# DakeQQ/Automatic-Speech-Recognition-ASR-ONNX

Hardware: AMD Instinct MI355X
Metric: audio-sec/s, SenseVoiceSmall, 8 s @ 16 kHz chunks, batch 64 per GPU (RTF = 1/value per GPU-stream) (higher is better)
Workload: dtype bf16; 1 GPU; SenseVoiceSmall bf16 (234 M params, 70 SANM blocks), batch=64 x 8 s per GPU, greedy CTC; step k's audio is resident in HBM when the step starts, batch k+1's host->device copy (pinned, copy stream) and every token-id download are inside the timed region; global_batch=64, parallelism=dp1 (utterance sharding, RCCL arena broadcast + hypothesis gather)

## Files before the change

automatic-speech-recognition-asr-onnx_amd/_lib.py:

```python
from __future__ import annotations

import ctypes as C
import os
import subprocess

_HERE = os.path.dirname(os.path.abspath(__file__))
LIB_PATH = os.path.join(_HERE, "libasr_mi355x.so")
CSRC_DIR = os.path.join(_HERE, "csrc")

_lib = None


class AsrError(RuntimeError):
    def __init__(self, code: int, message: str):
        super().__init__(f"[asr_mi355x status {code}] {message}")
        self.code = code


class SenseVoiceConfigC(C.Structure):
    _fields_ = [(n, C.c_int32) for n in (
        "sample_rate", "n_mels", "nfft", "win_length", "hop_length", "lfr_m", "lfr_n", "d_model", "n_heads", "d_head",
        "d_ffn", "n_blocks", "n_main", "fsmn_kernel", "vocab", "blank_id", "n_prompt", "n_languages", "max_audio_len")] + [
        ("reserved", C.c_int32 * 8)]

# ... 20 lines not shown


_vp, _i, _sz = C.c_void_p, C.c_int, C.c_size_t
_fp, _ip, _lp, _dp = C.POINTER(C.c_float), C.POINTER(C.c_int32), C.POINTER(C.c_int64), C.POINTER(C.c_double)
SIGNATURES = {
    "asr_abi_version": (_i, []),
    "asr_last_error": (C.c_char_p, []),
    "asr_device_count": (_i, [C.POINTER(C.c_int)]),
    "asr_device_foreign_begin": (_i, [_i]),
    "asr_device_foreign_end": (_i, [_i]),
    "asr_device_foreign_stats": (_i, [_i, _lp]),
    "asr_sensevoice_create": (_i, [C.POINTER(SenseVoiceConfigC), _vp, _sz, _i, _i, _i, C.POINTER(_vp)]),
    "asr_sensevoice_run": (_i, [_vp, _vp, _i, _lp, _i, _ip, _ip, _i, _ip]),
    "asr_sensevoice_run_timed": (_i, [_vp, _vp, _i, _lp, _i, _ip, _ip, _i, _ip, _ip, _ip, _fp]),
    "asr_sensevoice_run_beam": (_i, [_vp, _vp, _i, _lp, _i, _ip, _i, _i, _i, _ip, _i, _ip, _fp, _fp]),
    "asr_sensevoice_set_hotwords": (_i, [_vp, _ip, _ip, _i, C.c_float]),
    "asr_sensevoice_set_lm": (_i, [_vp, _ip, C.c_int64, C.c_float, C.c_float, C.c_float]),
    "asr_sensevoice_align": (_i, [_vp, _vp, _i, _lp, _i, _ip, _ip, _ip, _ip, _ip, _fp, _fp, _fp, _ip]),
    "asr_sanm_stats": (_i, [_vp, _ip]),
    "asr_sensevoice_seq_len": (_i, [C.POINTER(SenseVoiceConfigC), _i, C.POINTER(C.c_int)]),
    "asr_paraformer_create": (_i, [C.POINTER(ParaformerConfigC), _vp, _sz, _i, _i, _i, C.POINTER(_vp)]),
    "asr_paraformer_run": (_i, [_vp, _vp, _i, _lp, _i, _ip, _i, _ip]),
    "asr_paraformer_run_timed": (_i, [_vp, _vp, _i, _lp, _i, _ip, _i, _ip, _ip, _fp]),
    "asr_paraformer_run_beam": (_i, [_vp, _vp, _i, _lp, _i, _i, _i, _i, _ip, _i, _ip, _fp, _fp, _ip, _fp]),
    "asr_paraformer_set_hotwords": (_i, [_vp, _ip, _ip, _i, C.c_float]),
    "asr_paraformer_set_lm": (_i, [_vp, _ip, C.c_int64, C.c_float, C.c_float, C.c_float]),
    "asr_paraformer_stream_create": (_i, [C.POINTER(ParaformerConfigC), _vp, _sz, _i, _i, _i, _i, _i, _i, _i, C.POINTER(_vp)]),
    "asr_paraformer_stream_reset": (_i, [_vp, _i]),
    "asr_paraformer_stream_step": (_i, [_vp, _vp, _i, _ip, _i, _ip, _i, _ip]),
    "asr_paraformer_stream_step_timed": (_i, [_vp, _vp, _i, _ip, _i, _ip, _i, _ip, _ip, _fp]),
    "asr_paraformer_stream_set_beam": (_i, [_vp, _i, _i, _i, _i]),
    "asr_paraformer_stream_set_hotwords": (_i, [_vp, _ip, _ip, _i, C.c_float]),
    "asr_paraformer_stream_set_lm": (_i, [_vp, _ip, C.c_int64, C.c_float, C.c_float, C.c_float]),
    "asr_paraformer_stream_step_beam": (_i, [_vp, _vp, _i, _ip, _i, _ip, _i, _ip, _ip, _fp, _ip, _fp, _ip, _ip, _fp, _ip, _fp, _fp, _ip]),
    "asr_paraformer_stream_finish_beam": (_i, [_vp, _ip, _i, _ip, _fp, _ip, _ip, _fp, _ip, _fp, _fp, _ip]),
    "asr_paraformer_stream_stats": (_i, [_vp, _ip]),
    "asr_whisper_create": (_i, [C.POINTER(WhisperConfigC), _vp, _sz, _i, _i, _i, C.POINTER(_vp)]),
    "asr_whisper_encode": (_i, [_vp, _vp, _i, _lp, _i, _ip]),
    "asr_whisper_prefill": (_i, [_vp, _ip, _i, _ip, _fp]),
    "asr_whisper_prefill_prompts": (_i, [_vp, _ip, _ip, _ip, _fp]),
    "asr_whisper_decode": (_i, [_vp, _ip, _ip, _fp]),
    "asr_whisper_generate": (_i, [_vp, _i, _i, _ip, _ip]),
    "asr_whisper_beam_search": (_i, [_vp, _i, _i, _i, _ip, _ip, _fp]),
    "asr_whisper_set_penalty": (_i, [_vp, C.c_float, _i]),
    "asr_whisper_track_history": (_i, [_vp, _i]),
    "asr_whisper_set_fp8_act_shift": (_i, [_vp, _i]),
    "asr_whisper_fp8_stats": (_i, [_vp, C.POINTER(C.c_uint64)]),
    "asr_whisper_no_speech_prob": (_i, [_vp, _i, _fp]),
    "asr_whisper_set_sampling": (_i, [_vp, _i, C.c_float, _i, C.c_float, C.c_float, C.c_uint64]),
    "asr_whisper_set_sampling_noise": (_i, [_vp, _fp, _i]),
    "asr_whisper_set_timestamps": (_i, [_vp, _i, _i, _i, _i, _i]),
    "asr_whisper_set_token_scores": (_i, [_vp, _i]),
    "asr_whisper_set_hotwords": (_i, [_vp, _ip, _ip, _i, C.c_float]),
    "asr_whisper_set_lm": (_i, [_vp, _ip, C.c_int64, C.c_float, C.c_float, C.c_float, _i, _ip, _i]),
    "asr_whisper_token_scores": (_i, [_vp, _fp, _i, _ip]),
    "asr_whisper_set_word_timestamps": (_i, [_vp, _i, _ip, _i, _i]),
    "asr_whisper_align": (_i, [_vp, _ip, _ip, _i, _ip, _i]),
    "asr_whisper_align_read": (_i, [_vp, _i, _i, _vp, _sz, _ip]),
    "asr_qwen_create": (_i, [C.POINTER(QwenConfigC), _vp, _sz, _i, _i, _i, C.POINTER(_vp)]),
    "asr_qwen_prefill": (_i, [_vp, _vp, _i, _lp, _i, _ip, _ip, _ip, _ip, _ip, _fp, _ip]),
    "asr_qwen_decode": (_i, [_vp, _ip, _ip, _fp]),
    "asr_qwen_generate": (_i, [_vp, _i, _ip, _i, _ip, _ip]),
    "asr_qwen_kv_stats": (_i, [_vp, _ip]),
    "asr_qwen_beam_search": (_i, [_vp, _i, _i, _ip, _i, _ip, _ip, _fp]),
    "asr_qwen_set_penalty": (_i, [_vp, C.c_float, _i]),
    "asr_qwen_track_history": (_i, [_vp, _i]),
    "asr_qwen_set_sampling": (_i, [_vp, _i, C.c_float, _i, C.c_float, C.c_float, C.c_uint64]),
    "asr_qwen_set_sampling_noise": (_i, [_vp, _fp, _i]),
    "asr_qwen_set_token_scores": (_i, [_vp, _i]),
    "asr_qwen_set_hotwords": (_i, [_vp, _ip, _ip, _i, C.c_float]),
    "asr_qwen_set_lm": (_i, [_vp, _ip, C.c_int64, C.c_float, C.c_float, C.c_float, _i, _ip, _i]),
    "asr_qwen_token_scores": (_i, [_vp, _fp, _i, _ip]),
    "asr_qwen_align": (_i, [_vp, _vp, _i, _lp, _i, _ip, _ip, _ip, _ip, C.c_int32, _ip, _ip, C.c_int64, _fp, _ip]),
    "asr_mem_alloc": (_i, [_i, _sz, C.POINTER(_vp)]),
    "asr_mem_free": (_i, [_i, _vp]),
    "asr_mem_copy": (_i, [_i, _vp, _vp, _sz, _i]),
    "asr_session_destroy": (_i, [_vp]),
    "asr_session_set_stream": (_i, [_vp, _vp]),
    "asr_session_device": (_i, [_vp, C.POINTER(C.c_int)]),
    "asr_session_set_audio_dtype": (_i, [_vp, _i]),
    "asr_session_audio_dtype": (_i, [_vp, C.POINTER(C.c_int)]),
    "asr_session_set_input_format": (_i, [_vp, _i, _i]),
    "asr_session_input_format": (_i, [_vp, C.POINTER(C.c_int), C.POINTER(C.c_int)]),
    "asr_session_profile_enable": (_i, [_vp, _i]),
    "asr_session_profile_reset": (_i, [_vp]),
    "asr_session_profile_read": (_i, [_vp, _i, C.c_char_p, _dp, _lp, C.POINTER(C.c_int)]),
    "asr_session_taps_enable": (_i, [_vp, _i]),
    "asr_session_tap_shape": (_i, [_vp, C.c_char_p, _lp, _lp]),
    "asr_session_tap_read": (_i, [_vp, C.c_char_p, _vp, _sz]),
    "asr_op_gemm": (_i, [_i, _fp, _fp, _fp, _i, _i, _i, _i, _fp]),
    "asr_op_layernorm": (_i, [_i, _fp, _i, _i, _fp, _fp, C.c_float, _fp]),
    "asr_op_attention": (_i, [_i, _fp, _fp, _fp, _ip, _i, _i, _i, _fp]),
    "asr_op_fsmn": (_i, [_i, _fp, _fp, _fp, _ip, _i, _i, _i, _fp]),
    "asr_op_gemm_ln": (_i, [_fp, _fp, _fp, _fp, _fp, _i, _i, _i, _fp]),
    "asr_op_ctc_collapse": (_i, [_ip, _ip, _i, _i, _ip, _i, _ip]),
    "asr_op_ctc_collapse_timed": (_i, [_ip, _fp, _ip, _i, _i, _ip, _ip, _ip, _fp, _i, _ip]),
    "asr_op_ctc_prefix_beam": (_i, [_ip, _fp, _i, _ip, _i, _i, _ip, _ip, _ip, _ip, _ip, _i, C.c_float, _i, _i, _ip, _i, _ip, _fp, _fp]),
    "asr_op_ctc_prefix_beam_lm": (_i, [_ip, _fp, _i, _ip, _i, _i, _ip, _ip, _ip, _ip, _ip, _i, C.c_float, _i, _i, _ip, _i, _ip, _fp, _fp, _ip, C.c_int64, C.c_float,
                                       C.c_float, C.c_float]),
    "asr_op_nar_beam": (_i, [_ip, _fp, _i, _ip, _i, _ip, _ip, _ip, _ip, _ip, _i, C.c_float, _ip, C.c_int64, C.c_float, C.c_float, C.c_float, _i, _i, _ip, _i, _ip,
                             _fp, _fp, _fp]),
    "asr_nar_stream_beam_state_words": (_i, [_i, _i]),
    "asr_op_nar_stream_beam": (_i, [_ip, _fp, _i, _i, _i, _ip, _ip, _ip, _ip, _ip, _ip, _ip, _ip, _ip, _i, C.c_float, _ip, C.c_int64, C.c_float, C.c_float, C.c_float,
                                    _i, _i, _i, _ip, _i, _ip, _fp, _i, _ip, _ip, _fp, _ip, _fp, _fp, _ip]),
    "asr_op_ctc_align": (_i, [_fp, _i, _ip, _i, _i, _ip, _ip, _ip, _ip, _fp, _i, _fp, _fp, _ip]),
    "asr_op_cif_scan_timed": (_i, [_fp, _fp, _i, _ip, _i, C.c_float, _fp, _ip, _i, _ip]),
    "asr_op_resample": (_i, [_vp, _lp, _i, _i, _i, _i, _i, _i, _fp, C.c_int64, _lp]),
    "asr_resample_table": (_i, [_i, _i, C.POINTER(C.c_int), C.POINTER(C.c_int), C.POINTER(C.c_int), _fp]),
}


def build(force: bool = False) -> str:
    if force:
        subprocess.run(["make", "-C", CSRC_DIR, "clean"], check=True, capture_output=True)
    res = subprocess.run(["make", "-C", CSRC_DIR, "-j8"], capture_output=True, text=True)
    if res.returncode != 0:
        raise RuntimeError("building libasr_mi355x.so failed:\n" + res.stdout[-4000:] + res.stderr[-4000:])
    return LIB_PATH


def load():
    global _lib
    if _lib is not None:
        return _lib
    if not os.path.isfile(LIB_PATH):
        raise ImportError(f"{LIB_PATH} is missing: run `python -c 'import __graft_entry__ as g; g.build()'` "
                          "(the engine has no CPU fallback)")
    lib = C.CDLL(LIB_PATH, mode=C.RTLD_GLOBAL)
    for name, (res, args) in SIGNATURES.items():
        fn = getattr(lib, name)
        fn.restype = res
        fn.argtypes = args
    _lib = lib
    return lib


def check(status: int):
    if status != 0:
        raise AsrError(status, load().asr_last_error().decode("utf-8", "replace"))


def device_count() -> int:
    n = C.c_int(0)
    check(load().asr_device_count(C.byref(n)))
    return n.value
```

automatic-speech-recognition-asr-onnx_amd/csrc/api.hip:

```cpp
#include <cstring>

#include "../../include/asr_mi355x.h"
#include "engine.h"
#include "gemm.h"
#include "kernels.h"
#include "ngram_lm.h"

const std::string& asr_get_error();

extern "C" int asr_abi_version(void) { return ASR_ABI_VERSION; }
extern "C" const char* asr_last_error(void) { return asr_get_error().c_str(); }

extern "C" int asr_device_count(int* count) {
  return asr_guard([&] {
    ASR_REQUIRE(count, "device_count: null argument");
    int n = 0;
    if (hipGetDeviceCount(&n) != hipSuccess) n = 0;
    *count = n;
  });
}

extern "C" int asr_mem_alloc(int device_id, size_t bytes, void** out) {
  return asr_guard([&] {
    ASR_REQUIRE(out, "mem_alloc: null argument");
    asr_require_device(device_id);
    HIP_CHECK(hipMalloc(out, std::max<size_t>(bytes, 16)));
  });
}

extern "C" int asr_mem_free(int device_id, void* ptr) {
  return asr_guard([&] {
    if (!ptr) return;
    asr_require_device(device_id);
    HIP_CHECK(hipFree(ptr));
  });
}

extern "C" int asr_mem_copy(int device_id, void* dst, const void* src, size_t bytes, int kind) {
  return asr_guard([&] {
    ASR_REQUIRE(dst && src, "mem_copy: null argument");
    ASR_REQUIRE(kind >= 0 && kind <= 2, "mem_copy: bad kind %d", kind);
    asr_require_device(device_id);
    static const hipMemcpyKind kinds[3] = {hipMemcpyHostToDevice, hipMemcpyDeviceToHost, hipMemcpyDeviceToDevice};
    HIP_CHECK(hipMemcpy(dst, src, bytes, kinds[kind]));
  });
}

extern "C" int asr_session_destroy(asr_session* s) {
  return asr_guard([&] {
    if (!s) return;
    (void)hipSetDevice(s->device);
    if (s->stream) (void)hipStreamSynchronize(s->stream);
    delete s;
  });
}

extern "C" int asr_session_set_stream(asr_session* s, void* hip_stream) {
  return asr_guard([&] {
    ASR_REQUIRE(s, "set_stream: null session");
    HIP_CHECK(hipStreamSynchronize(s->stream));
    if (s->own_stream && s->stream) (void)hipStreamDestroy(s->stream);
    s->stream = reinterpret_cast<hipStream_t>(hip_stream);
    s->own_stream = false;
  });
}

extern "C" int asr_session_device(asr_session* s, int* device_id) {
  return asr_guard([&] {
    ASR_REQUIRE(s && device_id, "session_device: null argument");
    *device_id = s->device;
  });
}

extern "C" int asr_session_set_audio_dtype(asr_session* s, int audio_dtype) {
  return asr_guard([&] {
    ASR_REQUIRE(s, "set_audio_dtype: null session");
    ASR_REQUIRE(audio_dtype == ASR_AUDIO_F32 || audio_dtype == ASR_AUDIO_I16 || audio_dtype == ASR_AUDIO_F16,
                "set_audio_dtype: unknown audio dtype %d (0 = f32, 1 = int16, 2 = f16)", audio_dtype);
    s->audio_dtype = audio_dtype;
  });
}

extern "C" int asr_session_audio_dtype(asr_session* s, int* audio_dtype_out) {
  return asr_guard([&] {
    ASR_REQUIRE(s && audio_dtype_out, "audio_dtype: null argument");
    *audio_dtype_out = s->audio_dtype;
  });
}

extern "C" int asr_session_set_input_format(asr_session* s, int sample_rate, int channels) {
  return asr_guard([&] {
    ASR_REQUIRE(s, "set_input_format: null session");
    ASR_REQUIRE(channels >= 1 && channels <= 8, "input format: %d channels (1..8)", channels);
    (void)resample_design(sample_rate, s->model_rate);
    const bool off = sample_rate == s->model_rate && channels == 1;
    s->in_rate = off ? 0 : sample_rate;
    s->in_channels = channels;
  });
}

extern "C" int asr_session_input_format(asr_session* s, int* sample_rate_out, int* channels_out) {
  return asr_guard([&] {
    ASR_REQUIRE(s && sample_rate_out && channels_out, "input_format: null argument");
    *sample_rate_out = s->in_rate ? s->in_rate : s->model_rate;
    *channels_out = s->in_channels;
  });
}

extern "C" int asr_session_profile_enable(asr_session* s, int enable) {
  return asr_guard([&] {
    ASR_REQUIRE(s, "profile_enable: null session");
    s->prof.enabled = enable != 0;
  });
}

extern "C" int asr_session_profile_reset(asr_session* s) {
  return asr_guard([&] {
    ASR_REQUIRE(s, "profile_reset: null session");
    s->prof.reset();
  });
}

extern "C" int asr_session_profile_read(asr_session* s, int cap, char* names, double* total_ms, int64_t* launches, int* n_out) {
  return asr_guard([&] {
    ASR_REQUIRE(s && names && total_ms && launches && n_out, "profile_read: null argument");
    const int n = std::min<int>(cap, (int)s->prof.names.size());
    for (int i = 0; i < n; ++i) {
      memset(names + i * 32, 0, 32);
      strncpy(names + i * 32, s->prof.names[i].c_str(), 31);
      total_ms[i] = s->prof.total_ms[i];
      launches[i] = s->prof.launches[i];
    }
    *n_out = n;
  });
}

extern "C" int asr_session_taps_enable(asr_session* s, int enable) {
  return asr_guard([&] {
    ASR_REQUIRE(s, "taps_enable: null session");
    s->taps_enabled = enable != 0;
  });
}

extern "C" int asr_session_tap_shape(asr_session* s, const char* name, int64_t* rows, int64_t* cols) {
  return asr_guard([&] {
    ASR_REQUIRE(s && name && rows && cols, "tap_shape: null argument");
    auto it = s->taps.find(name);
    if (it == s->taps.end()) throw AsrError{ASR_ERR_NOT_FOUND, std::string("tap '") + name + "' not recorded (enable taps, then run)"};
    *rows = it->second.rows;
    *cols = it->second.cols;
  });
}

extern "C" int asr_session_tap_read(asr_session* s, const char* name, void* host_out, size_t bytes) {
  return asr_guard([&] {
    ASR_REQUIRE(s && name && host_out, "tap_read: null argument");
    auto it = s->taps.find(name);
    if (it == s->taps.end()) throw AsrError{ASR_ERR_NOT_FOUND, std::string("tap '") + name + "' not recorded (enable taps, then run)"};
    const Tap& t = it->second;
    const size_t need = (size_t)t.rows * t.cols * t.elt;
    ASR_REQUIRE(bytes == need, "tap_read: '%s' is %zu bytes, buffer is %zu", name, need, bytes);
    HIP_CHECK(hipSetDevice(s->device));
    HIP_CHECK(hipMemcpyAsync(host_out, t.buf.ptr, need, hipMemcpyDeviceToHost, s->stream));
    HIP_CHECK(hipStreamSynchronize(s->stream));
  });
}

namespace {

// ... 742 lines not shown
```

automatic-speech-recognition-asr-onnx_amd/csrc/engine.h:

```cpp
#pragma once
#include <algorithm>
#include <cstring>
#include <functional>
#include <map>
#include <string>
#include <vector>

#include "common.h"
#include "gemm.h"
#include "kernels.h"
#include "plan_layout.h"
#include "result_layout.h"

#define ASR_LOCAL __attribute__((visibility("hidden")))

enum { ARENA_F32 = 0, ARENA_BF16 = 1, ARENA_I32 = 2, ARENA_F16 = 3 };

struct TensorRef {
  void* ptr = nullptr;
  int dtype = 0;
  int ndim = 0;
  int64_t shape[4] = {0, 0, 0, 0};
  int64_t numel() const {
    int64_t n = 1;
// ... 86 lines not shown
  uint64_t h = 1469598103934665603ull;
  GraphKey& mix(uint64_t v) { h = (h ^ v) * 1099511628211ull; return *this; }
  GraphKey& mix(const void* p) { return mix((uint64_t)(uintptr_t)p); }
};

struct StepGraph {
  hipGraphExec_t exec = nullptr;
  uint64_t key = 0, eager_key = 0;
  StepGraph() = default;
  StepGraph(const StepGraph&) = delete;
  StepGraph& operator=(const StepGraph&) = delete;
  ~StepGraph() { drop(); }
  template <typename F> void run(hipStream_t s, bool graphable, uint64_t k, F&& enqueue) {
    if (graphable && exec && k == key) {
      HIP_CHECK(hipGraphLaunch(exec, s));
    } else if (graphable && k == eager_key) {
      capture(s, k, enqueue);
      HIP_CHECK(hipGraphLaunch(exec, s));
    } else {
      enqueue();
      if (graphable) eager_key = k;
    }
  }
  void drop();

 private:
  void capture(hipStream_t s, uint64_t k, const std::function<void()>& enqueue);
};

struct Profiler {
  bool enabled = false;
  std::vector<std::string> names;
  std::vector<double> total_ms;
  std::vector<int64_t> launches;
  struct Pending { int cls; hipEvent_t a, b; };
  std::vector<Pending> pending;
  std::vector<int> open;
  std::vector<hipEvent_t> pool;

  Profiler() = default;
  Profiler(const Profiler&) = delete;
  Profiler& operator=(const Profiler&) = delete;
  ~Profiler();
  int cls(const char* name);
  void begin(int c, hipStream_t s);
  void end(hipStream_t s);
  void collect();
  void reset();
  hipEvent_t get_event();
};

struct ProfScope {
  Profiler& p; hipStream_t s; bool on;
  ProfScope(Profiler& p_, const char* name, hipStream_t s_) : p(p_), s(s_), on(p_.enabled) { if (on) p.begin(p.cls(name), s); }
  ~ProfScope() { if (on) p.end(s); }
};

struct Tap {
  DeviceBuffer buf;
  int64_t rows = 0, cols = 0;
  int elt = 4;
};

struct Resampler {
  struct Table { ResampleDesign d; DeviceBuffer tab_t; };
  std::map<std::pair<int, int>, Table> tables;
  DeviceBuffer d_in, d_out, d_plan;
  PinnedBuffer h_plan;
  std::vector<int64_t> offs;
  const Table& table(int rate_in, int rate_model, hipStream_t s);
  const float* run(const void* audio, int audio_mem, int audio_dtype, int rate_in, int rate_model, int channels, float scale, const int64_t* offsets_in, int batch,
                   hipStream_t s);
};

struct asr_session {
  int kind = 0;
  int device = 0;
  int tenant_slot = -1;
  int precision = 0;
  int audio_dtype = 0;
  size_t audio_elt() const { return audio_dtype == 0 ? 4 : 2; }
  int model_rate = 16000;
  int in_rate = 0, in_channels = 1;
  Resampler resampler;
  hipStream_t stream = nullptr;
  bool own_stream = false;
  Arena arena;
  Profiler prof;
  bool taps_enabled = false;
  std::map<std::string, Tap> taps;
  virtual ~asr_session();
  void save_tap(const char* name, const void* src, int64_t rows, int64_t cols, int64_t ld_src, int elt);
};

struct FrontEnd {
  const float *dft = nullptr, *melp = nullptr;
  const void* dft_split = nullptr;
  int n_bin_tiles = 0, n_kchunks = 0, n_mels = 0, win = 0, hop = 0, whisper = 0;
  float log_floor = 0.0f;
  void init(int nfft, int win_, int hop_, int n_mels_, int whisper_, float log_floor_);
  void plan_utt(const char* family, int b, const int64_t* offs, int max_audio_len, UttPlan& p, int& frames, int& n_fb) const;
  FbankArgs args(const void* audio, int audio_dtype, const UttPlan* plan, const int32_t* blk_utt, const int32_t* blk_f0, float* mel_out, float* blk_max) const;
};
void fill_fbank_blocks(const UttPlan* plan, int B, int32_t* blk_utt, int32_t* blk_f0);
void fill_query_blocks(const UttPlan* plan, int n, int q_rows, int32_t* qb_utt, int32_t* qb_q0);
struct AudioIn {
  const void* audio; int mem; const int64_t* offs; int dtype;
  bool resampled;
};
AudioIn stage_input(asr_session& s, bool int16_unit_scale, const void* audio, int audio_mem, const int64_t* offs, int batch);
const void* stage_audio(asr_session& s, DeviceBuffer& d_audio, const AudioIn& in, int64_t first_sample, int64_t n_samples, bool* moved = nullptr);

struct SplitKGemm {
  static constexpr size_t WS_BYTES = (size_t)16 << 20;
  static constexpr int TICKETS = 4096;
  DeviceBuffer ws, cnt;
  void ensure(hipStream_t s) { if (!ws.ptr) { ws.reserve(WS_BYTES, s); cnt.reserve((size_t)TICKETS * 4, s); } }
  GemmArgs attach(const GemmArgs& g0, hipStream_t s);
  void run(const GemmArgs& g0, int precision, hipStream_t s);
};

struct LowBitWeights {
  struct Slot { const void** w; int N, K; };
  struct Entry { const unsigned char* w; const float* s; const unsigned char* s4; };
  DeviceBuffer d_w8, d_wscale, d_wdq;
  std::vector<Entry> e;
  int per_layer = 0;
  bool fp4 = false;
  void build(int n_layers, bool fp4_, const std::function<std::vector<Slot>(int)>& layer_slots, hipStream_t s);
  template <typename G> void select(G& g, int layer, int wi) const {
    const Entry& x = e[(size_t)layer * per_layer + wi];
    if (fp4) { g.W4 = x.w; g.w_scale4 = x.s4; }
    else { g.W8 = x.w; g.w_scale = x.s; }
  }
};

template <typename F>
int asr_guard(F&& f) {
  try {
    f();
    return ASR_OK;
  } catch (const AsrError& e) {
    asr_set_error(e.msg);
    return e.code;
  } catch (const std::exception& e) {
    asr_set_error(std::string("internal error: ") + e.what());
    return ASR_ERR_INVALID;
  }
}

void asr_require_device(int device_id);

void asr_tenant_attach(asr_session* s);
struct TenantScope { asr_session* s; explicit TenantScope(asr_session* s_); ~TenantScope(); };
int asr_tenant_live_others(const asr_session* s);
int asr_tenant_busy_others(const asr_session* s, double window_ms);

struct ClusterScope {
  int dev; bool ok;
  explicit ClusterScope(int device);
  ~ClusterScope();
};

void dump_phase_clocks(const DeviceBuffer& times, int n_workgroups, int first, int last, const char* const* names, const char* title, bool inside_a = false);
```

automatic-speech-recognition-asr-onnx_amd/csrc/engine.hip:

```cpp
#include "engine.h"

#include <algorithm>
#include <atomic>
#include <cstdio>
#include <cstring>

#include "../../include/asr_mi355x.h"

static thread_local std::string g_last_error;
void asr_set_error(const std::string& msg) { g_last_error = msg; }
const std::string& asr_get_error() { return g_last_error; }

void asr_require_device(int device_id) {
  int n = 0;
  hipError_t e = hipGetDeviceCount(&n);
  if (e != hipSuccess || n <= 0)
    throw AsrError{ASR_ERR_NO_DEVICE, "no HIP device visible: the MI355X engine has no CPU fallback"};
  if (device_id < 0 || device_id >= n)
    throw AsrError{ASR_ERR_INVALID, "device_id " + std::to_string(device_id) + " out of range (" + std::to_string(n) + " devices)"};
  HIP_CHECK(hipSetDevice(device_id));
}

static std::atomic<int64_t> g_live_bytes{0};
int64_t asr_live_device_bytes() { return g_live_bytes.load(); }
// ... 170 lines not shown

hipEvent_t Profiler::get_event() {
  if (!pool.empty()) {
    hipEvent_t e = pool.back();
    pool.pop_back();
    return e;
  }
  hipEvent_t e;
  HIP_CHECK(hipEventCreate(&e));
  return e;
}

void Profiler::begin(int c, hipStream_t s) {
  Pending p{c, get_event(), get_event()};
  HIP_CHECK(hipEventRecord(p.a, s));
  open.push_back((int)pending.size());
  pending.push_back(p);
}

void Profiler::end(hipStream_t s) {
  HIP_CHECK(hipEventRecord(pending[open.back()].b, s));
  open.pop_back();
}

void Profiler::collect() {
  for (auto& p : pending) {
    float ms = 0.f;
    HIP_CHECK(hipEventElapsedTime(&ms, p.a, p.b));
    total_ms[p.cls] += ms;
    launches[p.cls] += 1;
    pool.push_back(p.a);
    pool.push_back(p.b);
  }
  pending.clear();
}

void Profiler::reset() {
  for (auto& v : total_ms) v = 0.0;
  for (auto& v : launches) v = 0;
}

Profiler::~Profiler() {
  for (auto& p : pending) { (void)hipEventDestroy(p.a); (void)hipEventDestroy(p.b); }
  for (auto e : pool) (void)hipEventDestroy(e);
}

void asr_session::save_tap(const char* name, const void* src, int64_t rows, int64_t cols, int64_t ld_src, int elt) {
  if (!taps_enabled) return;
  Tap& t = taps[name];
  t.rows = rows;
  t.cols = cols;
  t.elt = elt;
  t.buf.reserve((size_t)rows * cols * elt, stream);
  HIP_CHECK(hipMemcpy2DAsync(t.buf.ptr, (size_t)cols * elt, src, (size_t)ld_src * elt, (size_t)cols * elt, (size_t)rows,
                             hipMemcpyDeviceToDevice, stream));
}

void FrontEnd::init(int nfft, int win_, int hop_, int n_mels_, int whisper_, float log_floor_) {
  n_bin_tiles = (nfft / 2 + 1 + 15) / 16;
  n_kchunks = win_ / 16;
  n_mels = n_mels_; win = win_; hop = hop_; whisper = whisper_; log_floor = log_floor_;
}

void FrontEnd::plan_utt(const char* family, int b, const int64_t* offs, int max_audio_len, UttPlan& p, int& frames, int& n_fb) const {
  const int64_t n = offs[b + 1] - offs[b];
  ASR_REQUIRE(n >= win, whisper ? "%s: utterance %d has %lld samples (< n_fft %d)" : "%s: utterance %d has %lld samples (< one %d-sample frame)", family, b, (long long)n, win);
  ASR_REQUIRE(n <= max_audio_len, "%s: utterance %d has %lld samples (> max_audio_len %d)", family, b, (long long)n, max_audio_len);
  p.audio_off = offs[b] - offs[0];
  p.n_samples = (int)n;
  p.n_frames = whisper ? (int)n / hop : ((int)n - win) / hop + 1;
  p.frame_off = frames;
  p.blk0 = n_fb;
  frames += p.n_frames;
  n_fb += (p.n_frames + 63) / 64;
}

FbankArgs FrontEnd::args(const void* audio, int audio_dtype, const UttPlan* plan, const int32_t* blk_utt, const int32_t* blk_f0, float* mel_out,
                         float* blk_max) const {
  FbankArgs fa;
  fa.audio = audio; fa.audio_dtype = audio_dtype; fa.plan = plan; fa.blk_utt = blk_utt; fa.blk_f0 = blk_f0; fa.dft_packed = dft; fa.mel_packed = melp;
  fa.mel_out = mel_out; fa.n_bin_tiles = n_bin_tiles; fa.n_kchunks = n_kchunks; fa.n_mel_tiles = n_mels / 16; fa.n_mels = n_mels;
  fa.win = win; fa.hop = hop; fa.log_floor = log_floor; fa.whisper = whisper; fa.blk_max = blk_max; fa.dft_split = dft_split;
  fa.log_at_floor = (float)(whisper ? std::log10((double)log_floor) : std::log((double)log_floor));
  return fa;
}

void fill_fbank_blocks(const UttPlan* plan, int B, int32_t* blk_utt, int32_t* blk_f0) {
  for (int b = 0, i = 0; b < B; ++b)
    for (int f0 = 0; f0 < plan[b].n_frames; f0 += 64) { blk_utt[i] = b; blk_f0[i++] = f0; }
}
void fill_query_blocks(const UttPlan* plan, int n, int q_rows, int32_t* qb_utt, int32_t* qb_q0) {
  for (int u = 0, i = 0; u < n; ++u)
    for (int q0 = 0; q0 < plan[u].T; q0 += q_rows) { qb_utt[i] = u; qb_q0[i++] = q0; }
}

const Resampler::Table& Resampler::table(int rate_in, int rate_model, hipStream_t s) {
  auto it = tables.find({rate_in, rate_model});
  if (it != tables.end()) return it->second;
  const ResampleDesign d = resample_design(rate_in, rate_model);
  std::vector<float> c((size_t)d.L * d.T), ct(c.size());
  resample_table(d, c.data());
  for (int p = 0; p < d.L; ++p)
    for (int k = 0; k < d.T; ++k) ct[(size_t)k * d.L + p] = c[(size_t)p * d.T + k];
  Table& t = tables[{rate_in, rate_model}];
  t.d = d;
  t.tab_t.reserve(ct.size() * 4, s);
  HIP_CHECK(hipMemcpyAsync(t.tab_t.ptr, ct.data(), ct.size() * 4, hipMemcpyHostToDevice, s));
  HIP_CHECK(hipStreamSynchronize(s));
  return t;
}

const float* Resampler::run(const void* audio, int audio_mem, int audio_dtype, int rate_in, int rate_model, int channels, float scale, const int64_t* offsets_in,
                            int batch, hipStream_t s) {
  ASR_REQUIRE(audio && offsets_in && batch >= 1, "resample: null argument");
  ASR_REQUIRE(channels >= 1 && channels <= 8, "input format: %d channels (1..8)", channels);
  const Table& tb = table(rate_in, rate_model, s);
  const ResampleDesign& d = tb.d;
  offs.assign((size_t)batch + 1, 0);
  int64_t n_tiles = 0;
  for (int b = 0; b < batch; ++b) {
    const int64_t n_in = offsets_in[b + 1] - offsets_in[b];
    ASR_REQUIRE(n_in >= 0 && n_in <= INT32_MAX, "resample: utterance %d has %lld frames", b, (long long)n_in);
    const int64_t n_out = resample_n_out(n_in, d);
    ASR_REQUIRE(n_out <= INT32_MAX, "resample: utterance %d has %lld samples at the model rate", b, (long long)n_out);
    offs[b + 1] = offs[b] + n_out;
    n_tiles += (n_out + d.tile - 1) / d.tile;
  }
  ASR_REQUIRE(n_tiles <= INT32_MAX, "resample: %lld tiles", (long long)n_tiles);
  PlanBlob pb(h_plan, d_plan);
  const auto s_utt = pb.add<RsUtt>(batch);
  const auto s_tile_utt = pb.add<int32_t>(std::max<int64_t>(n_tiles, 1)), s_tile_n0 = pb.add<int32_t>(std::max<int64_t>(n_tiles, 1));
  pb.commit(s);
  RsUtt* hu = pb.host(s_utt);
  int32_t *tile_utt = pb.host(s_tile_utt), *tile_n0 = pb.host(s_tile_n0);
  const int64_t base0 = offsets_in[0];
  for (int b = 0, i = 0; b < batch; ++b) {
    hu[b].in_off = offsets_in[b] - base0; hu[b].out_off = offs[b];
    hu[b].n_in = (int32_t)(offsets_in[b + 1] - offsets_in[b]); hu[b].n_out = (int32_t)(offs[b + 1] - offs[b]);
    for (int n0 = 0; n0 < hu[b].n_out; n0 += d.tile) { tile_utt[i] = b; tile_n0[i++] = n0; }
  }
  pb.upload(s);
  const size_t frame_bytes = (size_t)channels * audio_elt_bytes(audio_dtype), in_bytes = (size_t)(offsets_in[batch] - base0) * frame_bytes;
  const void* src = static_cast<const unsigned char*>(audio) + (size_t)base0 * frame_bytes;
  if (audio_mem == ASR_MEM_HOST) {
    d_in.reserve(std::max<size_t>(in_bytes, 16), s);
    if (in_bytes) HIP_CHECK(hipMemcpyAsync(d_in.ptr, src, in_bytes, hipMemcpyHostToDevice, s));
    src = d_in.ptr;
  }
  d_out.reserve(std::max<size_t>((size_t)offs[batch] * 4, 16), s);
  ResampleArgs a;
  a.audio = src; a.utt = pb.dev(s_utt); a.tile_utt = pb.dev(s_tile_utt); a.tile_n0 = pb.dev(s_tile_n0); a.tab_t = tb.tab_t.as<float>(); a.out = d_out.as<float>();
  a.d = d; a.channels = channels; a.scale = scale; a.audio_dtype = audio_dtype;
  launch_resample(a, (int)n_tiles, s);
  return d_out.as<float>();
}

AudioIn stage_input(asr_session& s, bool int16_unit_scale, const void* audio, int audio_mem, const int64_t* offs, int batch) {
  if (!s.in_rate) return AudioIn{audio, audio_mem, offs, s.audio_dtype, false};
  ProfScope ps(s.prof, "resample", s.stream);
  const float scale = s.audio_dtype == AUDIO_I16 && int16_unit_scale ? 0x1p-15f : 1.0f;
  const float* out = s.resampler.run(audio, audio_mem, s.audio_dtype, s.in_rate, s.model_rate, s.in_channels, scale, offs, batch, s.stream);
  if (s.resampler.offs[batch] > 0) s.save_tap("resampled", out, 1, s.resampler.offs[batch], s.resampler.offs[batch], 4);
  return AudioIn{out, ASR_MEM_DEVICE, s.resampler.offs.data(), AUDIO_F32, true};
}

const void* stage_audio(asr_session& s, DeviceBuffer& d_audio, const AudioIn& in, int64_t first_sample, int64_t n_samples, bool* moved) {
  const size_t eA = audio_elt_bytes(in.dtype);
  const void* audio = in.audio;
  const int audio_mem = in.mem;
  const void* src = static_cast<const unsigned char*>(audio) + (size_t)first_sample * eA;
  void* before = d_audio.ptr;
  if (audio_mem == ASR_MEM_HOST) {
// ... 171 lines not shown
```

automatic-speech-recognition-asr-onnx_amd/csrc/kernels.h:

```cpp
#pragma once
#include <vector>

#include "common.h"
#include "ngram_lm.h"

struct UttPlan {
  int64_t audio_off;
  int32_t n_samples;
  int32_t n_frames;
  int32_t frame_off;
  int32_t n_lfr;
  int32_t T;
  int32_t row_off;
  int32_t lang;
  int32_t blk0;
};

enum { AUDIO_F32 = 0, AUDIO_I16 = 1, AUDIO_F16 = 2 };
inline size_t audio_elt_bytes(int audio_dtype) { return audio_dtype == AUDIO_F32 ? 4 : 2; }
struct FbankArgs {
  const void* audio;
  const UttPlan* plan;
  const int32_t* blk_utt;
  const int32_t* blk_f0;
  const float* dft_packed;
  const float* mel_packed;
  float* mel_out;
  int n_bin_tiles;
  int n_kchunks;
  int n_mel_tiles;
  int n_mels;
  int win, hop;
  float log_floor;
  int whisper;
  int dbg = 0;
  float* blk_max;
  const void* dft_split = nullptr;
  float log_at_floor = 0.0f;
  int audio_dtype = AUDIO_F32;
};
void launch_fbank(const FbankArgs& a, int n_blocks, hipStream_t s);
size_t fbank_split_table_bytes(int n_bin_tiles, int win);
void launch_fbank_split_table(const float* dft_packed, int n_bin_tiles, int n_kchunks16, void* out, hipStream_t s);

struct ResampleDesign {
  int L, M, W, T;
  int tile;
  int span_max;
};
ResampleDesign resample_design(int rate_in, int rate_model);
void resample_table(const ResampleDesign& d, float* coeffs);
inline int64_t resample_n_out(int64_t n_in, const ResampleDesign& d) { return (n_in * d.L + d.M - 1) / d.M; }
struct RsUtt {
  int64_t in_off;
  int64_t out_off;
  int32_t n_in, n_out;
};
struct ResampleArgs {
  const void* audio;
  const RsUtt* utt;
  const int32_t* tile_utt;
  const int32_t* tile_n0;
  const float* tab_t;
  float* out;
  ResampleDesign d;
  int channels;
  float scale;
  int audio_dtype = AUDIO_F32;
};
void launch_resample(const ResampleArgs& a, int n_tiles, hipStream_t s);

template <typename T>
void launch_whisper_mel_finish(const float* mel, const float* blk_max, const UttPlan* plan, const int32_t* grow_utt,
                               int n_gapped_rows, int n_mels, T* out, hipStream_t s);
void launch_compact_rows(const float* src, const UttPlan* from, const UttPlan* to, const int32_t* row_utt, int rows, int d, float* dst, hipStream_t s);
template <typename T>
void launch_zero_gap_rows(T* buf, int ld, int n_cols, const UttPlan* plan, const int32_t* grow_utt, int n_gapped_rows,
                          hipStream_t s);

void launch_layernorm_fp8(const float* x, int ld_x, int rows, int D, float eps, float inv_scale, unsigned char* out, int ld_out, hipStream_t s);

template <typename T>
void launch_embed_pos(const int32_t* ids, int rows, int n, int hist, const int32_t* hist_dev, const T* embed, const float* pos, int d,
                      float* x, hipStream_t s, const int32_t* kstart = nullptr, int kstart_rows = 0);
void launch_add_scalar(int32_t* p, int v, hipStream_t s);

struct DecAttnArgs {
  const void* q; int ld_q; int q_col0;
  const void* kv_new; int ld_new; int k_col0, v_col0;
  void* k_base; void* v_base;
  int64_t stride_b, stride_h;
  const UttPlan* plan;
  int hist, n, n_heads, causal;
  int max_keys = 0;
  int sc_ld = 0;
  const int32_t* hist_dev;
  void* out; int ld_out;
  const float* k_scale = nullptr; const float* v_scale = nullptr;
  const int32_t* page_table = nullptr; int pages_per_seq = 0; int64_t page_stride = 0;
  int b0 = 0, scale_ld = 0;
  const int32_t* beam_src = nullptr; int ld_src = 0, beam_p0 = 0, beam = 1;
  const int32_t* key_start = nullptr;
};

struct PromptAttnArgs {
  const void* q = nullptr; int ld_q = 0, q_col0 = 0;
  const void* kv_new = nullptr; int ld_new = 0, k_col0 = 0, v_col0 = 0;
  void* k_base = nullptr; void* v_base = nullptr;
  int64_t stride_b = 0, stride_h = 0;
  const int32_t* page_table = nullptr; int pages_per_seq = 0; int64_t page_stride = 0;
  const UttPlan* plan = nullptr;
  const int32_t* key_start = nullptr;
  int n = 0, n_heads = 0;
  void* out = nullptr; int ld_out = 0;
};
template <typename T>
void launch_prompt_attention(const PromptAttnArgs& a, int batch, hipStream_t s);
void launch_quantize_rows_fp8(const bf16_t* W, int ld, int N, int K, unsigned char* W8, float* scale, bf16_t* Wdq, hipStream_t s);
void launch_quantize_rows_mxfp4(const bf16_t* W, int ld, int N, int K, unsigned char* W4, unsigned char* S, bf16_t* Wdq, hipStream_t s);
void launch_quantize_crosskv_fp8(bf16_t* slabs, size_t slab_elems, int n_slabs, const UttPlan* plan, int batch, unsigned char* out8, float* scale,
                                 int dq_in_place, hipStream_t s);
// ... 349 lines not shown
```

automatic-speech-recognition-asr-onnx_amd/csrc/kernels.hip:

```cpp
#include "kernels.h"
#include "gemm.h"
#include "hot_trie.h"
#include "pcm.h"

#include <algorithm>
#include <type_traits>
#include <cstdlib>

namespace {

constexpr int HOP = 160, WIN = 400;
constexpr int FB_FRAMES = 64;
constexpr int FB_SPAN = (FB_FRAMES - 1) * HOP + WIN;
constexpr int FB_AUDIO_LDS = FB_SPAN + FB_SPAN / HOP + 16;
constexpr int FB_PLD = 273;

template <typename S>
__global__ __launch_bounds__(256) void fbank_kernel(const FbankArgs a) {
  extern __shared__ __attribute__((aligned(16))) unsigned char smem[];
  float* aud = reinterpret_cast<float*>(smem);
  float* pw = aud + FB_AUDIO_LDS;
  const int tid = threadIdx.x, lane = tid & 63, wave = tid >> 6;
  const int u = a.blk_utt[blockIdx.x], f0 = a.blk_f0[blockIdx.x];
  const UttPlan up = a.plan[u];
// ... 11 lines not shown
      idx = p < half ? half - p : p < half + L ? p - half : 2 * L + half - 2 - p;
      ok = i < FB_SPAN && p < L + WIN - HOP;
    }
    av[j] = ok ? Pcm<S>::load(src, idx) : (typename Pcm<S>::raw_t)0;
  }
#pragma unroll
  for (int j = 0; j < NL; ++j) av[j] = Pcm<S>::hold(av[j]);
#pragma unroll
  for (int j = 0; j < NL; ++j) {
    const int i = tid + j * 256;
    if (i < FB_SPAN) aud[i + i / HOP] = Pcm<S>::widen(av[j], pcm_scale);
  }
  __syncthreads();

  const int frow = lane & 15, fgrp = lane >> 4;
  const float4* dft = reinterpret_cast<const float4*>(a.dft_packed);
  for (int t = wave; t < a.n_bin_tiles; t += 4) {
    f32x4_t re[4], im[4];
#pragma unroll
    for (int mt = 0; mt < 4; ++mt) { re[mt] = f32x4_t{0.f, 0.f, 0.f, 0.f}; im[mt] = f32x4_t{0.f, 0.f, 0.f, 0.f}; }
    const float4* dre = dft + (size_t)(t * 2 + 0) * a.n_kchunks * 64 + lane;
    const float4* dim = dft + (size_t)(t * 2 + 1) * a.n_kchunks * 64 + lane;
    float4 br = dre[0], bi = dim[0];
    for (int kc = 0; kc < a.n_kchunks; ++kc) {
      float4 brn = br, bin = bi;
      if (kc + 1 < a.n_kchunks) { brn = dre[(kc + 1) * 64]; bin = dim[(kc + 1) * 64]; }
      const float brv[4] = {br.x, br.y, br.z, br.w};
      const float biv[4] = {bi.x, bi.y, bi.z, bi.w};
#pragma unroll
      for (int j = 0; j < 4; ++j) {
        const int k = kc * 16 + j * 4 + fgrp;
        const int koff = k + k / HOP;
        float af[4];
#pragma unroll
        for (int mt = 0; mt < 4; ++mt) af[mt] = aud[(mt * 16 + frow) * (HOP + 1) + koff];
#pragma unroll
        for (int mt = 0; mt < 4; ++mt) {
          re[mt] = __builtin_amdgcn_mfma_f32_16x16x4f32(af[mt], brv[j], re[mt], 0, 0, 0);
          im[mt] = __builtin_amdgcn_mfma_f32_16x16x4f32(af[mt], biv[j], im[mt], 0, 0, 0);
        }
      }
      br = brn; bi = bin;
    }
#pragma unroll
    for (int mt = 0; mt < 4; ++mt)
#pragma unroll
      for (int r = 0; r < 4; ++r)
        pw[(mt * 16 + fgrp * 4 + r) * FB_PLD + t * 16 + frow] = re[mt][r] * re[mt][r] + im[mt][r] * im[mt][r];
  }
  __syncthreads();

  float wmax = -INFINITY;
  const float4* melp = reinterpret_cast<const float4*>(a.mel_packed);
  for (int nt = 0; nt < a.n_mel_tiles; ++nt) {
    f32x4_t acc = f32x4_t{0.f, 0.f, 0.f, 0.f};
    float4 b4 = melp[(size_t)(nt * a.n_bin_tiles) * 64 + lane];
    for (int kc = 0; kc < a.n_bin_tiles; ++kc) {
      float4 b4n = b4;
      if (kc + 1 < a.n_bin_tiles) b4n = melp[(size_t)(nt * a.n_bin_tiles + kc + 1) * 64 + lane];
      const float bv[4] = {b4.x, b4.y, b4.z, b4.w};
#pragma unroll
      for (int j = 0; j < 4; ++j) {
        const float av = pw[(wave * 16 + frow) * FB_PLD + kc * 16 + j * 4 + fgrp];
        acc = __builtin_amdgcn_mfma_f32_16x16x4f32(av, bv[j], acc, 0, 0, 0);
      }
      b4 = b4n;
    }
#pragma unroll
    for (int r = 0; r < 4; ++r) {
      const int f = f0 + wave * 16 + fgrp * 4 + r;
      if (f < up.n_frames) {
        const float c = fmaxf(acc[r], a.log_floor);
        const float v = c <= a.log_floor ? a.log_at_floor : a.whisper ? log10f(c) : logf(c);
        a.mel_out[(size_t)(up.frame_off + f) * a.n_mels + nt * 16 + frow] = v;
        wmax = fmaxf(wmax, v);
      }
    }
  }
  if (a.whisper) {
    __shared__ float red[4];
    wmax = wave_max(wmax);
    if (lane == 0) red[wave] = wmax;
    __syncthreads();
    if (tid == 0) a.blk_max[blockIdx.x] = fmaxf(fmaxf(red[0], red[1]), fmaxf(red[2], red[3]));
  }
}

constexpr int FB_HP = HOP + 8;
constexpr int FB_K32 = (WIN + 31) / 32;
constexpr int FB_A16 = ((FB_SPAN + 32 + HOP - 1) / HOP) * FB_HP;

constexpr int FB_WAVES = 8;
template <typename S>
__global__ __launch_bounds__(64 * FB_WAVES) void fbank_split_kernel(const FbankArgs a) {
  extern __shared__ __attribute__((aligned(16))) unsigned char smem[];
  bf16_t* audh = reinterpret_cast<bf16_t*>(smem);
  bf16_t* audl = audh + FB_A16;
  float* pw = reinterpret_cast<float*>(audl + FB_A16);
  const int tid = threadIdx.x, lane = tid & 63, wave = tid >> 6;
  const int u = a.blk_utt[blockIdx.x], f0 = a.blk_f0[blockIdx.x];
  const UttPlan up = a.plan[u];
  const S* src = static_cast<const S*>(a.audio) + up.audio_off;
  const float pcm_scale = a.whisper ? 0x1p-15f : 1.0f;
  const int s0 = f0 * HOP;
  constexpr int FB_NL = (FB_SPAN + 32 + 64 * FB_WAVES - 1) / (64 * FB_WAVES);
  typename Pcm<S>::raw_t av[FB_NL];
#pragma unroll
  for (int j = 0; j < FB_NL; ++j) {
    const int i = tid + j * 64 * FB_WAVES;
    const int L = up.n_samples, half = WIN / 2, p = s0 + i;
    int idx = p;
    bool ok = i < FB_SPAN + 32 && p < L;
    if (a.whisper) {
      idx = p < half ? half - p : p < half + L ? p - half : 2 * L + half - 2 - p;
      ok = i < FB_SPAN + 32 && p < L + WIN - HOP;
    }
    av[j] = (ok && !(a.dbg & 4)) ? Pcm<S>::load(src, idx) : (typename Pcm<S>::raw_t)0;
  }
#pragma unroll
  for (int j = 0; j < FB_NL; ++j) av[j] = Pcm<S>::hold(av[j]);
#pragma unroll
  for (int j = 0; j < FB_NL; ++j) {
    const int i = tid + j * 64 * FB_WAVES;
    if (i < FB_SPAN + 32) {
      const float v = Pcm<S>::widen(av[j], pcm_scale);
      const uint32_t hb = pack_bf16x2(v, 0.0f) & 0xffffu;
      const float hi = __uint_as_float(hb << 16);
      const int pos = i + (i / HOP) * 8;
      audh[pos] = (bf16_t)hb;
      audl[pos] = (bf16_t)(pack_bf16x2(v - hi, 0.0f) & 0xffffu);
    }
  }
  __syncthreads();

  const int frow = lane & 15, fgrp = lane >> 4;
  const uint4* tab = reinterpret_cast<const uint4*>(a.dft_split);
  constexpr int FB_PF = 4;
  union BF { uint4 q; bf16x8_t v; };
  BF ring[FB_PF][6];
  const int wv = __builtin_amdgcn_readfirstlane(wave);
  const int n_steps = (wv < a.n_bin_tiles && !(a.dbg & 1)) ? (a.n_bin_tiles - wv + FB_WAVES - 1) / FB_WAVES * FB_K32 : 0;
  constexpr size_t FB_IM = (size_t)FB_K32 * 3 * 64;
  auto frag_ptr = [&](int t, int kc) { return tab + (((size_t)(t * 2) * FB_K32 + kc) * 3) * 64 + lane; };
  int pt = wv, pkc = 0, ps = 0;
  auto refill = [&](BF (&slot)[6]) {
    const uint4* src = frag_ptr(pt, pkc);
#pragma unroll
    for (int z = 0; z < 3; ++z) { slot[z].q = src[z * 64]; slot[3 + z].q = src[FB_IM + z * 64]; }
    if (ps + 1 < n_steps) { ++ps; if (++pkc == FB_K32) { pkc = 0; pt += FB_WAVES; } }
  };
  f32x4_t re[4], im[4];
#pragma unroll
  for (int mt = 0; mt < 4; ++mt) { re[mt] = f32x4_t{0.f, 0.f, 0.f, 0.f}; im[mt] = f32x4_t{0.f, 0.f, 0.f, 0.f}; }
  if (n_steps > 0) {
#pragma unroll
    for (int u = 0; u < FB_PF; ++u) refill(ring[u]);
  }
  int t = wv, kc = 0;
  for (int s0 = 0; s0 < n_steps; s0 += FB_PF) {
#pragma unroll
    for (int u = 0; u < FB_PF; ++u) {
      if (s0 + u < n_steps) {
        const int k = kc * 32 + fgrp * 8;
        const int koff = k + ((k >= HOP) + (k >= 2 * HOP)) * 8;
        bf16x8_t ah[4], al[4];
#pragma unroll
        for (int mt = 0; mt < 4; ++mt) {
          const int pos = (mt * 16 + frow) * FB_HP + koff;
          ah[mt] = *reinterpret_cast<const bf16x8_t*>(audh + pos); al[mt] = *reinterpret_cast<const bf16x8_t*>(audl + pos);
        }
#define ASR_FB_TERM(X, ZR, ZI)                                                                          \
        _Pragma("unroll") for (int mt = 0; mt < 4; ++mt) {                                               \
          re[mt] = __builtin_amdgcn_mfma_f32_16x16x32_bf16(X[mt], ring[u][ZR].v, re[mt], 0, 0, 0);       \
          im[mt] = __builtin_amdgcn_mfma_f32_16x16x32_bf16(X[mt], ring[u][ZI].v, im[mt], 0, 0, 0);       \
        }
        ASR_FB_TERM(al, 1, 4)
        ASR_FB_TERM(ah, 2, 5)
        ASR_FB_TERM(al, 0, 3)
        ASR_FB_TERM(ah, 1, 4)
        ASR_FB_TERM(ah, 0, 3)
#undef ASR_FB_TERM
        if (++kc == FB_K32) {
#pragma unroll
          for (int mt = 0; mt < 4; ++mt) {
#pragma unroll
            for (int r = 0; r < 4; ++r)
              pw[(mt * 16 + fgrp * 4 + r) * FB_PLD + t * 16 + frow] = re[mt][r] * re[mt][r] + im[mt][r] * im[mt][r];
            re[mt] = f32x4_t{0.f, 0.f, 0.f, 0.f}; im[mt] = f32x4_t{0.f, 0.f, 0.f, 0.f};
          }
          kc = 0; t += FB_WAVES;
        }
      }
      __builtin_amdgcn_sched_barrier(0);
      if (!(a.dbg & 8)) refill(ring[u]);
      __builtin_amdgcn_sched_barrier(0);
    }
  }
  __syncthreads();

  float wmax = -INFINITY;
  const float4* melp = reinterpret_cast<const float4*>(a.mel_packed);
  constexpr int FB_MT = 4;
  const int fw = wave & 3, mg = wave >> 2;
  for (int nt0 = mg; nt0 < ((a.dbg & 2) ? 0 : a.n_mel_tiles); nt0 += 2 * FB_MT) {
    f32x4_t acc[FB_MT];
#pragma unroll
    for (int q = 0; q < FB_MT; ++q) acc[q] = f32x4_t{0.f, 0.f, 0.f, 0.f};
    auto mel_frags = [&](float4 (&b)[FB_MT], int kc) {
#pragma unroll
      for (int q = 0; q < FB_MT; ++q) b[q] = nt0 + 2 * q < a.n_mel_tiles ? melp[(size_t)((nt0 + 2 * q) * a.n_bin_tiles + kc) * 64 + lane] : make_float4(0.f, 0.f, 0.f, 0.f);
    };
    float4 b4[FB_MT], b4n[FB_MT];
    mel_frags(b4, 0);
    for (int kc = 0; kc < a.n_bin_tiles; ++kc) {
      mel_frags(b4n, kc + 1 < a.n_bin_tiles ? kc + 1 : kc);
#pragma unroll
      for (int j = 0; j < 4; ++j) {
        const float av = pw[(fw * 16 + frow) * FB_PLD + kc * 16 + j * 4 + fgrp];
#pragma unroll
        for (int q = 0; q < FB_MT; ++q) {
          const float bv = j == 0 ? b4[q].x : j == 1 ? b4[q].y : j == 2 ? b4[q].z : b4[q].w;
          if (nt0 + 2 * q < a.n_mel_tiles) acc[q] = __builtin_amdgcn_mfma_f32_16x16x4f32(av, bv, acc[q], 0, 0, 0);
        }
      }
#pragma unroll
      for (int q = 0; q < FB_MT; ++q) b4[q] = b4n[q];
    }
#pragma unroll
    for (int q = 0; q < FB_MT; ++q) {
      if (nt0 + 2 * q >= a.n_mel_tiles) continue;
#pragma unroll
      for (int r = 0; r < 4; ++r) {
        const int f = f0 + fw * 16 + fgrp * 4 + r;
        if (f < up.n_frames) {
          const float c = fmaxf(acc[q][r], a.log_floor);
          const float v = c <= a.log_floor ? a.log_at_floor : a.whisper ? log10f(c) : logf(c);
          a.mel_out[(size_t)(up.frame_off + f) * a.n_mels + (nt0 + 2 * q) * 16 + frow] = v;
          wmax = fmaxf(wmax, v);
        }
      }
    }
  }
  if (a.whisper) {
    __shared__ float red[FB_WAVES];
    wmax = wave_max(wmax);
    if (lane == 0) red[wave] = wmax;
    __syncthreads();
    if (tid == 0) {
      float m = red[0];
#pragma unroll
      for (int w = 1; w < FB_WAVES; ++w) m = fmaxf(m, red[w]);
      a.blk_max[blockIdx.x] = m;
    }
  }
}

__global__ void fbank_split_table_kernel(const float* __restrict__ dft_packed, int n_bin_tiles, int n_kchunks16, uint4* __restrict__ out) {
  const int idx = blockIdx.x * blockDim.x + threadIdx.x;
  const int total = n_bin_tiles * 2 * FB_K32 * 64;
  if (idx >= total) return;
  const int lane = idx & 63, kc = (idx >> 6) % FB_K32, tr = (idx >> 6) / FB_K32;
  const int frow = lane & 15, fgrp = lane >> 4;
  uint32_t w[3][4] = {};
  for (int e = 0; e < 8; ++e) {
    const int k = kc * 32 + fgrp * 8 + e;
    float v = 0.0f;
    if (k < n_kchunks16 * 16) {
      v = dft_packed[(((size_t)tr * n_kchunks16 + (k >> 4)) * 64 + ((k & 3) * 16 + frow)) * 4 + ((k & 15) >> 2)];
    }
    float r = v;
    for (int z = 0; z < 3; ++z) {
      const uint32_t b = pack_bf16x2(r, 0.0f) & 0xffffu;
      r -= __uint_as_float(b << 16);
      w[z][e >> 1] |= b << ((e & 1) * 16);
    }
  }
  for (int z = 0; z < 3; ++z) out[((size_t)(tr * FB_K32 + kc) * 3 + z) * 64 + lane] = make_uint4(w[z][0], w[z][1], w[z][2], w[z][3]);
}

__global__ void lfr_cmvn_kernel(const LfrArgs a) {
  const int m = blockIdx.x;
  float* o = a.out + (size_t)m * a.ld_out;
  const int u = a.row_utt[m];
  bf16_t* olo = a.out_lo ? a.out_lo + (size_t)m * a.ld_out : nullptr;
  if (u < 0) {
    for (int c = threadIdx.x; c < a.ld_out; c += blockDim.x) { o[c] = 0.0f; if (olo) olo[c] = 0; }
    return;
  }
  const UttPlan up = a.plan[u];
  const int t = m - up.row_off;
  const int left = (a.lfr_m - 1) / 2;
  for (int c = threadIdx.x; c < a.ld_out; c += blockDim.x) {
    float v = 0.0f;
    if (c < a.feat && t < up.T) {
      if (a.n_prompt > 0 && t == 0) {
        v = a.language_embed[(size_t)up.lang * a.feat + c];
      } else if (t < a.n_prompt) {
        v = a.system_embed[(size_t)(t - 1) * a.feat + c];
      } else {
        const int j = t - a.n_prompt;
        int f = j * a.lfr_n + c / a.n_mels - left;
        f = min(max(f, 0), up.n_frames - 1);
        const float x = a.mel[(size_t)(up.frame_off + f) * a.n_mels + c % a.n_mels];
        if (a.affine_mode == 1) {
          v = x * a.cmvn_vars[c] + a.speech_pos[(size_t)j * a.feat + c];
        } else {
          v = (x + a.cmvn_means[c]) * a.cmvn_vars[c];
          v = v + a.speech_pos[(size_t)j * a.feat + c];
        }
      }
    }
    o[c] = v;
    if (olo) olo[c] = f32_to_bf16(v);
  }
}

constexpr int LN_MAXV = 8;
template <typename OutT>
__global__ __launch_bounds__(256) void layernorm_kernel(const float* __restrict__ x, int ld_x, int rows, int D,
                                                        const float* __restrict__ gamma, const float* __restrict__ beta,
                                                        float eps, OutT* out, int ld_out, int fill_to, const int32_t* __restrict__ rows_dev,
                                                        bf16_t* out_lo, int ld_lo) {
  const int row = blockIdx.x * 4 + (threadIdx.x >> 6);
  const int lane = threadIdx.x & 63;
  if (row >= rows || (rows_dev && row >= *rows_dev)) return;
  const float* xr = x + (size_t)row * ld_x;
  float4 v[LN_MAXV];
  float s = 0.0f;
#pragma unroll
  for (int k = 0; k < LN_MAXV; ++k) {
    const int i = k * 256 + lane * 4;
    v[k] = (i < D) ? *reinterpret_cast<const float4*>(xr + i) : make_float4(0.f, 0.f, 0.f, 0.f);
    s += (v[k].x + v[k].y) + (v[k].z + v[k].w);
  }
  const float mean = wave_sum(s) / (float)D;
// ... 1162 lines not shown

__global__ __launch_bounds__(256) void fsmn_rows_kernel(const float* __restrict__ x, const float* __restrict__ res, const float* __restrict__ w,
                                                        int d, int ktaps, const UttPlan* __restrict__ tplan,
                                                        const int32_t* __restrict__ row_utt, float* __restrict__ out,
                                                        const int32_t* __restrict__ rows_dev) {
  const int m = blockIdx.x;
  if (rows_dev && m >= *rows_dev) return;
  const int u = row_utt[m];
  int s = 0, e = 0;
  if (u >= 0) { s = tplan[u].row_off; e = s + tplan[u].T; }
  const int pad = (ktaps - 1) / 2;
  for (int c = threadIdx.x; c < d; c += blockDim.x) {
    float acc = 0.f;
    if (m >= s && m < e) {
      acc = res[(size_t)m * d + c];
      for (int j = 0; j < ktaps; ++j) {
        const int mm = m + j - pad;
        if (mm >= s && mm < e) acc = fmaf(w[c * ktaps + j], x[(size_t)mm * d + c], acc);
      }
    }
    out[(size_t)m * d + c] = acc;
  }
}

__global__ __launch_bounds__(256) void token_compact_kernel(const UttPlan* __restrict__ own, int n_utts, int n_rows_max,
                                                            UttPlan* __restrict__ compact, int32_t* __restrict__ row_utt,
                                                            int32_t* __restrict__ total_rows) {
  __shared__ int total_s;
  if (threadIdx.x == 0) {
    int off = 0;
    for (int u = 0; u < n_utts; ++u) {
      UttPlan tp = own[u];
      tp.row_off = off;
      compact[u] = tp;
      off += (tp.T + 15) & ~15;
    }
    total_s = off;
    *total_rows = off;
  }
  __syncthreads();
  const int total = total_s;
  for (int r = threadIdx.x; r < n_rows_max; r += 256) row_utt[r] = -1;
  __syncthreads();
  for (int u = 0; u < n_utts; ++u) {
    const int r0 = compact[u].row_off, n16 = (compact[u].T + 15) & ~15;
    for (int r = threadIdx.x; r < n16; r += 256)
      if (r0 + r < min(total, n_rows_max)) row_utt[r0 + r] = u;
  }
}

__global__ __launch_bounds__(256) void compact_rows_kernel(const float* __restrict__ src, const UttPlan* __restrict__ own,
                                                           const UttPlan* __restrict__ compact, int d, float* __restrict__ dst) {
  const int u = blockIdx.x, s0 = own[u].row_off, d0 = compact[u].row_off, n16 = (compact[u].T + 15) & ~15;
  for (int e = threadIdx.x; e < n16 * d; e += 256) dst[(size_t)d0 * d + e] = src[(size_t)s0 * d + e];
}

__global__ void gather_tokens_kernel(const int32_t* __restrict__ ids, const UttPlan* __restrict__ tplan, int32_t* __restrict__ token_ids,
                                     int max_tokens) {
  const int u = blockIdx.x;
  const int n = min(tplan[u].n_lfr, max_tokens);
  for (int i = threadIdx.x; i < n; i += blockDim.x) token_ids[(size_t)u * max_tokens + i] = ids[tplan[u].row_off + i];
}

__global__ void gather_token_logprob_kernel(const float* __restrict__ row_logprob, const UttPlan* __restrict__ tplan,
                                            float* __restrict__ token_logprob, int max_tokens) {
  const int u = blockIdx.x;
  const int n = min(tplan[u].n_lfr, max_tokens);
  for (int i = threadIdx.x; i < n; i += blockDim.x) token_logprob[(size_t)u * max_tokens + i] = row_logprob[tplan[u].row_off + i];
}

}

template <typename S>
static void launch_fbank_typed(const FbankArgs& a, int n_blocks, hipStream_t s) {
  ASR_REQUIRE(a.win == WIN && a.hop == HOP, "fbank: only win=400 hop=160 is built (got %d/%d)", a.win, a.hop);
  ASR_REQUIRE(a.n_bin_tiles * 16 <= FB_PLD - 1, "fbank: too many frequency bins");
  ASR_REQUIRE(a.n_kchunks * 16 == WIN, "fbank: k-chunks must cover the window");
  const size_t lds = (size_t)(FB_AUDIO_LDS + FB_FRAMES * FB_PLD) * sizeof(float);
  static PerDeviceOnce attr_once;
  if (attr_once.first()) {
    HIP_CHECK(hipFuncSetAttribute(reinterpret_cast<const void*>(fbank_kernel<S>), hipFuncAttributeMaxDynamicSharedMemorySize, (int)lds));
  }
  if (a.dft_split) {
    FbankArgs b = a;
    b.dbg = env_int("ASR_FBANK_DBG", b.dbg);
    const size_t lds2 = (size_t)FB_A16 * 2 * 2 + (size_t)FB_FRAMES * FB_PLD * sizeof(float);
    static PerDeviceOnce attr2_once;
    if (attr2_once.first()) {
      HIP_CHECK(hipFuncSetAttribute(reinterpret_cast<const void*>(fbank_split_kernel<S>), hipFuncAttributeMaxDynamicSharedMemorySize, (int)lds2));
    }
    hipLaunchKernelGGL(fbank_split_kernel<S>, dim3(n_blocks), dim3(64 * FB_WAVES), lds2, s, b);
    HIP_CHECK(hipGetLastError());
    return;
  }
  hipLaunchKernelGGL(fbank_kernel<S>, dim3(n_blocks), dim3(256), lds, s, a);
  HIP_CHECK(hipGetLastError());
}
void launch_fbank(const FbankArgs& a, int n_blocks, hipStream_t s) {
  switch (a.audio_dtype) {
    case AUDIO_F32: return launch_fbank_typed<float>(a, n_blocks, s);
    case AUDIO_I16: return launch_fbank_typed<int16_t>(a, n_blocks, s);
    case AUDIO_F16: return launch_fbank_typed<_Float16>(a, n_blocks, s);
    default: ASR_THROW(ASR_ERR_INVALID, "fbank: unknown audio sample type %d", a.audio_dtype);
  }
}

size_t fbank_split_table_bytes(int n_bin_tiles, int win) {
  ASR_REQUIRE(win == WIN, "fbank: only win=400 is built (got %d)", win);
  return (size_t)n_bin_tiles * 2 * FB_K32 * 3 * 64 * 16;
}
void launch_fbank_split_table(const float* dft_packed, int n_bin_tiles, int n_kchunks16, void* out, hipStream_t s) {
  const int total = n_bin_tiles * 2 * FB_K32 * 64;
  hipLaunchKernelGGL(fbank_split_table_kernel, dim3((total + 255) / 256), dim3(256), 0, s, dft_packed, n_bin_tiles, n_kchunks16, reinterpret_cast<uint4*>(out));
  HIP_CHECK(hipGetLastError());
}

void launch_lfr_cmvn(const LfrArgs& a, hipStream_t s) {
  hipLaunchKernelGGL(lfr_cmvn_kernel, dim3(a.n_rows), dim3(256), 0, s, a);
  HIP_CHECK(hipGetLastError());
}

template <typename OutT>
void launch_layernorm(const float* x, int ld_x, int rows, int D, const float* gamma, const float* beta, float eps,
                      OutT* out, int ld_out, int fill_to, hipStream_t s, const int32_t* rows_dev) {
  ASR_REQUIRE(D % 4 == 0 && D <= LN_MAXV * 256 && ld_x % 4 == 0 && ld_out % 4 == 0, "layernorm: D=%d ld=%d unsupported", D, ld_x);
  hipLaunchKernelGGL(layernorm_kernel<OutT>, dim3((rows + 3) / 4), dim3(256), 0, s, x, ld_x, rows, D, gamma, beta, eps, out,
                     ld_out, fill_to, rows_dev, (bf16_t*)nullptr, 0);
  HIP_CHECK(hipGetLastError());
}
void launch_layernorm_with_bf16_copy(const float* x, int ld_x, int rows, int D, const float* gamma, const float* beta, float eps,
                                     float* out, int ld_out, bf16_t* out_lo, int ld_lo, hipStream_t s) {
  ASR_REQUIRE(D % 4 == 0 && D <= LN_MAXV * 256 && ld_x % 4 == 0 && ld_out % 4 == 0 && ld_lo % 4 == 0 && out_lo, "layernorm: D=%d ld=%d unsupported", D, ld_x);
  hipLaunchKernelGGL(layernorm_kernel<float>, dim3((rows + 3) / 4), dim3(256), 0, s, x, ld_x, rows, D, gamma, beta, eps, out, ld_out, D, (const int32_t*)nullptr, out_lo, ld_lo);
  HIP_CHECK(hipGetLastError());
}
template void launch_layernorm<float>(const float*, int, int, int, const float*, const float*, float, float*, int, int, hipStream_t, const int32_t*);
template void launch_layernorm<bf16_t>(const float*, int, int, int, const float*, const float*, float, bf16_t*, int, int, hipStream_t, const int32_t*);

void launch_layernorm_fp8(const float* x, int ld_x, int rows, int D, float eps, float inv_scale, unsigned char* out, int ld_out, hipStream_t s) {
  ASR_REQUIRE(D % 256 == 0 && D <= 2048 && ld_x % 4 == 0 && ld_out % 4 == 0, "layernorm_fp8: D=%d unsupported", D);
  hipLaunchKernelGGL(layernorm_fp8_kernel, dim3((rows + 3) / 4), dim3(256), 0, s, x, ld_x, rows, D, eps, inv_scale, out, ld_out);
  HIP_CHECK(hipGetLastError());
}

static thread_local AttnLaunchInfo g_attn_launch;
const AttnLaunchInfo& attention_last_launch() { return g_attn_launch; }

template <int HD, int CHUNK, int QT>
static void launch_attn_inst(const AttnArgs& a, hipStream_t s) {
  constexpr int lds = CHUNK * HD * 2 * 2;
  g_attn_launch = AttnLaunchInfo{HD, CHUNK, QT, a.n_waves, 0};
  static PerDeviceOnce attr_once;
  if (attr_once.first()) {
    HIP_CHECK(hipFuncSetAttribute(reinterpret_cast<const void*>(attn_bf16_kernel<HD, CHUNK, QT>),
                                  hipFuncAttributeMaxDynamicSharedMemorySize, lds));
  }
  AttnArgs b = a;
  if (b.ld_q == 0) b.ld_q = b.ld_qk;
  hipLaunchKernelGGL((attn_bf16_kernel<HD, CHUNK, QT>), dim3(a.n_qblocks, a.n_heads), dim3(64 * a.n_waves), lds, s, b, a.ld_vt);
  HIP_CHECK(hipGetLastError());
}

void attention_geometry(int max_T, int head_dim, int* qt, int* nw) {
  const int qt_max = 2;
  const int n_tiles = (max_T + 15) / 16;
  int q = 1;
  while (q < qt_max && (n_tiles + q - 1) / q > 8) ++q;
  q = std::max(1, std::min(qt_max, env_int("ASR_ATTN_QT", q)));
  int w = std::min(8, (n_tiles + q - 1) / q);
  w = std::max(1, std::min(8, env_int("ASR_ATTN_NW", w)));
  *qt = q;
  *nw = w;
}

void launch_attention_bf16_hd128(const AttnArgs& a, hipStream_t s) {
  ASR_REQUIRE(a.qt >= 1 && a.qt <= 2 && a.n_waves >= 1 && a.n_waves <= 8, "attention: bad geometry qt=%d nw=%d", a.qt, a.n_waves);
  const bool big = a.max_T <= 256;
  if (a.qt == 1) { big ? launch_attn_inst<128, 256, 1>(a, s) : launch_attn_inst<128, 128, 1>(a, s); }
  else { big ? launch_attn_inst<128, 256, 2>(a, s) : launch_attn_inst<128, 128, 2>(a, s); }
}
void launch_attention_bf16_hd64(const AttnArgs& a, hipStream_t s) {
  ASR_REQUIRE(a.qt >= 1 && a.qt <= 2 && a.n_waves >= 1 && a.n_waves <= 8, "attention: bad geometry qt=%d nw=%d", a.qt, a.n_waves);
  if (a.qt == 1) launch_attn_inst<64, 256, 1>(a, s); else launch_attn_inst<64, 256, 2>(a, s);
}

void launch_attention_f32(const AttnArgs& a, int head_dim, hipStream_t s) {
  ASR_REQUIRE(head_dim <= 128 && head_dim % 4 == 0, "attention_f32: head_dim %d unsupported", head_dim);
// ... 1182 lines not shown
```

automatic-speech-recognition-asr-onnx_amd/csrc/qwen.hip:

```cpp
#include <cstdlib>
#include <cstring>
#include <type_traits>
#include <vector>

#include "../../include/asr_mi355x.h"
#include "decode_head.h"
#include "engine.h"
#include "gemm.h"
#include "kernels.h"
#include "qwen_attn.h"

namespace {

inline int round_up(int v, int m) { return (v + m - 1) / m * m; }

inline int feat_lengths(int n) {
  const int leave = n % 100;
  const int f1 = leave > 0 ? (std::max(leave - 1, 0) / 2 + 1) : 0;
  const int f2 = f1 > 0 ? (std::max(f1 - 1, 0) / 2 + 1) : 0;
  const int f3 = f2 > 0 ? (std::max(f2 - 1, 0) / 2 + 1) : 0;
  return f3 + (n / 100) * 13;
}

inline size_t pad_rows(size_t r) { return (r + 127) / 128 * 128 + 144; }
// ... 556 lines not shown
  int vpad = 0, hpad = 0, cpad = 0, chunk = 0, cpw = 0, rpw = 0, t_tok = 13;
  std::vector<QwEncLayer> enc;
  std::vector<QwDecLayer> dec;
  FrontEnd fe;
  const float *conv1_b = nullptr, *conv2_b = nullptr, *conv3_b = nullptr, *enc_pos = nullptr,
              *proj1_b = nullptr, *proj2_b = nullptr, *rope = nullptr, *final_norm = nullptr;
  const void *conv1_w = nullptr, *conv2_w = nullptr, *conv3_w = nullptr, *conv_out_w = nullptr, *proj1_w = nullptr, *proj2_w = nullptr,
             *embed = nullptr, *lm_head = nullptr;
  int batch = 0;
  std::vector<int> seq_len;
  DeviceBuffer d_plan, d_audio, d_mel, d_blkmax, d_feat, d_col, d_c1, d_c2, d_c3, d_xa, d_xb, d_h, d_qk, d_vt, d_ctx, d_ffn, d_aud_out;
  std::vector<char> frozen;
  DeviceBuffer d_dplan, d_x, d_x2, d_dh, d_qkv, d_q, d_dctx, d_act, d_last, d_logits, d_next, d_kc, d_vc, d_hist, d_stepplan, d_vt2, d_krows, d_xlo, d_x2lo;
  bool no_fuse = false, use_graph = true;
  bool fp4 = false;
  bool fp8 = false, fp8_fake = false;
  bool use_decode_gemm = true;
  LowBitWeights dec8;
  bool kv_paged = true, kv_shuffle = false;
  int kv_pps = 0, kv_pool_pages = 0, kv_high_water = 0;
  std::vector<int32_t> kv_free, kv_table;
  std::vector<std::vector<int32_t>> kv_owned;
  std::vector<char> kv_released;
  DeviceBuffer d_kvtab;
  PinnedBuffer h_kvtab;
  bool kv_table_dirty = false;
  size_t kv_page_elems() const { return (size_t)cfg.n_layers * cfg.n_kv_heads * 16 * cfg.d_head; }
  void kv_begin(int B, const std::vector<int>& lens, size_t eT);
  void kv_prepare_step(size_t eT);
  int kv_take(size_t eT);
  void kv_upload();
  KvAddr kv_addr() const {
    if (kv_paged) return KvAddr{d_kvtab.as<int32_t>(), kv_pps, kv_page_elems(), cfg.max_seq_len};
    return KvAddr{nullptr, 0, 0, cfg.max_seq_len};
  }
  TokenHead head;
  DeviceBuffer d_sel, d_amax_v, d_amax_i, d_bucket;
  DeviceBuffer d_bkc, d_bvc, d_bhist, d_bp0, d_bplan;
  BeamRanker ranker;
  StepGraph dec_graph;
  PinnedBuffer h_plan, h_stepplan, h_io, h_ids;
  SplitKGemm sk;
  void gemm(const GemmArgs& g) { sk.run(g, precision, stream); }
  DecPass step_plan(DeviceBuffer& dev, int rows);
  DecPass step_pass;
  void init();
  bool aligner() const { return cfg.classify_num > 0; }
  template <typename T> void prefill(const void* audio, int audio_mem, const int64_t* offs, int B, const int32_t* pre_ids, const int32_t* pre_off,
                                     const int32_t* post_ids, const int32_t* post_off, int32_t* next_out, float* logits_out, int32_t* ids_len_out,
                                     const AlignReq* al = nullptr);
  template <typename T> void align_head(int B, const UttPlan* ddp, const int32_t* d_src, int n_sel, const AlignReq& al);
  template <typename T> void decoder_pass(const DecPass& P);
  template <typename T> void logits_head(const DecPass& P);
  template <typename T> void step(const int32_t* ids_host, int32_t* next_out, float* logits_out);
  void finish(int B, int32_t* next_out, float* logits_out, bool sync);
  template <typename T> void beam_search(int beam, int max_new, const int32_t* stop_ids, int n_stop, int32_t* tokens_out, int32_t* n_out, float* scores_out);
};

void QwSession::init() {
  const auto& c = cfg;
  ASR_REQUIRE(c.nfft == 400 && c.hop_length == 160 && c.n_mels == 128, "qwen: front-end is built for n_fft 400 / hop 160 / 128 mels");
  ASR_REQUIRE(c.d_head == 128 && c.n_heads % c.n_kv_heads == 0, "qwen: decoder head_dim must be 128");
  ASR_REQUIRE(c.enc_d % 128 == 0 && c.enc_d / c.enc_heads == 64 && c.enc_ffn % 128 == 0, "qwen: encoder needs 64-wide heads and widths that are multiples of 128");
  ASR_REQUIRE(c.d_model % 128 == 0 && c.d_ffn % 64 == 0 && (2 * c.d_ffn) % 128 == 0, "qwen: decoder widths must be multiples of 128");
  ASR_REQUIRE(c.n_window == 50, "qwen: the conv stem is built for 100-frame chunks (n_window 50)");
  chunk = 2 * c.n_window;
  cpw = c.n_window_infer / chunk;
  rpw = round_up(cpw * t_tok, 16);
  ASR_REQUIRE(cpw >= 1 && rpw <= 1024, "qwen: bad attention window");
  vpad = round_up(c.vocab, 128);
  head.init(c.max_seq_len, 1, 10, 1024);
  head.prof = &prof; ranker.prof = &prof;
  ASR_REQUIRE(c.classify_num >= 0, "qwen: classify_num %d", c.classify_num);
  hpad = aligner() ? round_up(c.classify_num, 128) : vpad;
  cpad = round_up(c.conv_channels, 128);
  fe.init(c.nfft, c.nfft, c.hop_length, c.n_mels, 1, 1e-10f);
  model_rate = c.sample_rate;
  const int wt = precision == ASR_PRECISION_BF16 ? ARENA_BF16 : ARENA_F32;
  const int de = c.enc_d, d = c.d_model, qkvn = (c.n_heads + 2 * c.n_kv_heads) * c.d_head;
  auto F = [&](const std::string& n, std::initializer_list<int64_t> sh) { return (const float*)arena.get(n, ARENA_F32, sh).ptr; };
  auto W = [&](const std::string& n, std::initializer_list<int64_t> sh) { return arena.get(n, wt, sh).ptr; };
  fe.dft = F("fe.dft", {(int64_t)fe.n_bin_tiles * 2 * fe.n_kchunks * 64 * 4});
  fe.melp = F("fe.mel", {(int64_t)(c.n_mels / 16) * fe.n_bin_tiles * 64 * 4});
  conv1_w = W("enc.conv1_w", {cpad, 64});          conv1_b = F("enc.conv1_b", {cpad});
  conv2_w = W("enc.conv2_w", {cpad, 9 * cpad});    conv2_b = F("enc.conv2_b", {cpad});
  conv3_w = W("enc.conv3_w", {cpad, 9 * cpad});    conv3_b = F("enc.conv3_b", {cpad});
  conv_out_w = W("enc.conv_out_w", {de, 16 * cpad});
  enc_pos = F("enc.pos", {t_tok, de});
  enc.resize(c.n_enc_layers);
  for (int i = 0; i < c.n_enc_layers; ++i) {
    const std::string q = "enc" + std::to_string(i) + ".";
    enc[i] = {W(q + "wqkv", {3 * de, de}), W(q + "wo", {de, de}), W(q + "w1", {c.enc_ffn, de}), W(q + "w2", {de, c.enc_ffn}),
              F(q + "bqkv", {3 * de}), F(q + "bo", {de}), F(q + "b1", {c.enc_ffn}), F(q + "b2", {de})};
  }
  proj1_w = W("enc.proj1_w", {de, de});   proj1_b = F("enc.proj1_b", {de});
  proj2_w = W("enc.proj2_w", {d, de});    proj2_b = F("enc.proj2_b", {d});
  embed = W("dec.embed", {vpad, d});
  lm_head = W("dec.lm_head", {hpad, d});
  rope = F("dec.rope", {c.max_seq_len, c.d_head});
  final_norm = F("dec.final_norm", {d});
  dec.resize(c.n_layers);
  for (int i = 0; i < c.n_layers; ++i) {
    const std::string q = "dec" + std::to_string(i) + ".";
    dec[i] = {W(q + "wqkv", {qkvn, d}), W(q + "wo", {d, c.n_heads * c.d_head}), W(q + "gate_up", {2 * c.d_ffn, d}), W(q + "down", {d, c.d_ffn}),
              F(q + "qn", {c.d_head}), F(q + "kn", {c.d_head})};
  }
  if (fp8) {
    const int I = c.d_ffn, od = c.n_heads * c.d_head;
    ASR_REQUIRE(d % 256 == 0 && I % 256 == 0 && od % 256 == 0, "qwen: FP8 mode needs d_model, d_ffn and heads x head_dim to be multiples of 256");
    dec8.build(c.n_layers, fp4, [&](int i) {
      QwDecLayer& L = dec[i];
      return std::vector<LowBitWeights::Slot>{{&L.wqkv, qkvn, d}, {&L.wo, d, od}, {&L.gate_up, 2 * I, d}, {&L.down, d, I}};
    }, stream);
    HIP_CHECK(hipStreamSynchronize(stream));
  }
}

void QwSession::kv_upload() {
  if (!kv_table_dirty) return;
  const size_t bytes = kv_table.size() * 4;
  h_kvtab.reserve(bytes);
  int32_t* st = h_kvtab.as<int32_t>();
  memcpy(st, kv_table.data(), bytes);
  HIP_CHECK(hipMemcpyAsync(d_kvtab.ptr, st, bytes, hipMemcpyHostToDevice, stream));
  HIP_CHECK(hipStreamSynchronize(stream));
  kv_table_dirty = false;
}
int QwSession::kv_take(size_t eT) {
  if (kv_free.empty()) {
    const int old_pages = kv_pool_pages, new_pages = std::max(2 * old_pages, old_pages + 64);
    DeviceBuffer nk, nv;
    nk.reserve((size_t)new_pages * kv_page_elems() * eT, stream);
    nv.reserve((size_t)new_pages * kv_page_elems() * eT, stream);
    HIP_CHECK(hipMemcpyAsync(nk.ptr, d_kc.ptr, (size_t)old_pages * kv_page_elems() * eT, hipMemcpyDeviceToDevice, stream));
    HIP_CHECK(hipMemcpyAsync(nv.ptr, d_vc.ptr, (size_t)old_pages * kv_page_elems() * eT, hipMemcpyDeviceToDevice, stream));
    HIP_CHECK(hipStreamSynchronize(stream));
    d_kc = std::move(nk); d_vc = std::move(nv);
    for (int p = new_pages - 1; p >= old_pages; --p) kv_free.push_back(p);
    kv_pool_pages = new_pages;
  }
  const int p = kv_free.back();
  kv_free.pop_back();
  kv_high_water = std::max(kv_high_water, kv_pool_pages - (int)kv_free.size());
  return p;
}
void QwSession::kv_begin(int B, const std::vector<int>& lens, size_t eT) {
  const auto& c = cfg;
  kv_pps = (c.max_seq_len + 15) / 16;
  auto prompt_pages = [&](int len) { return std::min((len + 1 + 15) / 16, kv_pps); };
  int need = 1;
  for (int b = 0; b < B; ++b) need += prompt_pages(lens[b]);
  if (need > kv_pool_pages) {
    d_kc.release(); d_vc.release();
    d_kc.reserve((size_t)need * kv_page_elems() * eT, stream);
    d_vc.reserve((size_t)need * kv_page_elems() * eT, stream);
    kv_pool_pages = need;
  }
  kv_free.clear();
  for (int p = kv_pool_pages - 1; p >= 1; --p) kv_free.push_back(p);
  if (kv_shuffle) {
    uint64_t x = 0x9e3779b97f4a7c15ull;
    for (size_t i = kv_free.size(); i > 1; --i) { x ^= x << 13; x ^= x >> 7; x ^= x << 17; std::swap(kv_free[i - 1], kv_free[x % i]); }
  }
  kv_table.assign((size_t)B * kv_pps, 0);
  kv_owned.assign(B, {});
  kv_released.assign(B, 0);
// ... 753 lines not shown
```

automatic-speech-recognition-asr-onnx_amd/csrc/sensevoice.hip:

```cpp
#include <cmath>
#include <cstdlib>
#include <cstring>

#include "sanm_session.h"

void SvSession::init() {
  const auto& c = cfg;
  ASR_REQUIRE(c.d_model == c.n_heads * c.d_head, "sensevoice: d_model != n_heads * d_head");
  ASR_REQUIRE(c.d_model % 128 == 0 && c.d_ffn % 128 == 0, "sensevoice: d_model and d_ffn must be multiples of 128");
  ASR_REQUIRE(c.d_head == 128 || (precision == ASR_PRECISION_F32 && c.d_head <= 128), "sensevoice: head_dim %d unsupported", c.d_head);
  ASR_REQUIRE(c.win_length == 400 && c.hop_length == 160, "sensevoice: front-end is built for 25 ms / 10 ms frames");
  ASR_REQUIRE(c.n_mels % 16 == 0, "sensevoice: n_mels must be a multiple of 16");
  ASR_REQUIRE(c.n_blocks >= 1 && c.n_main >= 1 && c.n_main <= c.n_blocks, "sensevoice: bad block counts");
  auto opt = [&](const std::string& n, std::initializer_list<int64_t> sh) -> const float* {
    return arena.has(n) ? (const float*)arena.get(n, ARENA_F32, sh).ptr : nullptr;
  };
  feat = c.n_mels * c.lfr_m;
  kpad0 = round_up(feat, 64);
  vpad = round_up(c.vocab, 128);
  fe.init(c.nfft, c.win_length, c.hop_length, c.n_mels, 0, 1.1920928955078125e-07f);
  model_rate = c.sample_rate;
  const int n_frames_max = (c.max_audio_len - c.win_length) / c.hop_length + 1;
  max_lfr = (n_frames_max + c.lfr_n - 1) / c.lfr_n;
  const int wt = precision == ASR_PRECISION_BF16 ? ARENA_BF16 : ARENA_F32;
  const int d = c.d_model, dff = c.d_ffn;

  fe.dft = (const float*)arena.get("fe.dft", ARENA_F32, {(int64_t)fe.n_bin_tiles * 2 * fe.n_kchunks * 64 * 4}).ptr;
  if (precision == ASR_PRECISION_BF16 && use_fbank_split) {
    d_dft_split.reserve(fbank_split_table_bytes(fe.n_bin_tiles, cfg.win_length), stream);
    launch_fbank_split_table(fe.dft, fe.n_bin_tiles, fe.n_kchunks, d_dft_split.ptr, stream);
    HIP_CHECK(hipStreamSynchronize(stream));
    fe.dft_split = d_dft_split.ptr;
  }
  fe.melp = (const float*)arena.get("fe.mel", ARENA_F32, {(int64_t)(c.n_mels / 16) * fe.n_bin_tiles * 64 * 4}).ptr;
  cmvn_means = opt("fe.cmvn_means", {feat});
  cmvn_vars = (const float*)arena.get("fe.cmvn_vars", ARENA_F32, {feat}).ptr;
  speech_pos = (const float*)arena.get("fe.speech_pos", ARENA_F32, {max_lfr, feat}).ptr;
  language_embed = c.n_prompt > 0 ? (const float*)arena.get("fe.language_embed", ARENA_F32, {c.n_languages, feat}).ptr : nullptr;
  system_embed = c.n_prompt > 1 ? (const float*)arena.get("fe.system_embed", ARENA_F32, {c.n_prompt - 1, feat}).ptr : nullptr;
  after_g = (const float*)arena.get("after_norm_g", ARENA_F32, {d}).ptr;
  after_b = (const float*)arena.get("after_norm_b", ARENA_F32, {d}).ptr;
  if (!paraformer) {
    tp_g = (const float*)arena.get("tp_norm_g", ARENA_F32, {d}).ptr;
    tp_b = (const float*)arena.get("tp_norm_b", ARENA_F32, {d}).ptr;
    ctc_w = arena.get("ctc.w", wt, {vpad, d}).ptr;
    ctc_b = (const float*)arena.get("ctc.b", ARENA_F32, {vpad}).ptr;
  } else {
    const int dd = pcfg.d_dec_ffn;
    ASR_REQUIRE(dd % 128 == 0 && dd <= 2048 && (3 * d) % 64 == 0 && pcfg.cif_kernel == 3, "paraformer: unsupported decoder geometry");
    cif_conv_w = arena.get("cif.conv_w", wt, {d, 3 * d}).ptr;
    cif_conv_b = (const float*)arena.get("cif.conv_b", ARENA_F32, {d}).ptr;
    cif_out_w = (const float*)arena.get("cif.out_w", ARENA_F32, {d}).ptr;
    cif_out_b = (const float*)arena.get("cif.out_b", ARENA_F32, {1}).ptr;
    pf_out_w = arena.get("out.w", wt, {vpad, d}).ptr;
    pf_out_b = (const float*)arena.get("out.b", ARENA_F32, {vpad}).ptr;
    pdec.resize(pcfg.n_dec + pcfg.n_dec3);
    for (int j = 0; j < (int)pdec.size(); ++j) {
      PfDecLayer& L = pdec[j];
      const std::string q = "dec" + std::to_string(j) + ".";
      L.full = j < pcfg.n_dec;
      L.w1 = arena.get(q + "w1", wt, {dd, d}).ptr;
      L.b1 = (const float*)arena.get(q + "b1", ARENA_F32, {dd}).ptr;
      L.w2 = arena.get(q + "w2", wt, {d, dd}).ptr;
      L.b2 = (const float*)arena.get(q + "b2", ARENA_F32, {d}).ptr;
      if (L.full) {
        L.n2_g = (const float*)arena.get(q + "n2_g", ARENA_F32, {d}).ptr;
        L.n2_b = (const float*)arena.get(q + "n2_b", ARENA_F32, {d}).ptr;
        L.wfsmn = (const float*)arena.get(q + "wfsmn", ARENA_F32, {d, c.fsmn_kernel}).ptr;
        L.wq = arena.get(q + "wq", wt, {d, d}).ptr;
        L.bq = (const float*)arena.get(q + "bq", ARENA_F32, {d}).ptr;
        L.wkv = arena.get(q + "wkv", wt, {2 * d, d}).ptr;
        L.bkv = (const float*)arena.get(q + "bkv", ARENA_F32, {2 * d}).ptr;
        L.wo = arena.get(q + "wo", wt, {d, d}).ptr;
        L.bo = (const float*)arena.get(q + "bo", ARENA_F32, {d}).ptr;
      }
    }
    pf_kv_batch = env_flag("ASR_PF_KV_BATCH", pf_kv_batch);
    pf_n_full = 0;
    for (const PfDecLayer& L : pdec) pf_n_full += L.full ? 1 : 0;
    if (pf_kv_batch && pf_n_full > 0) {
      const size_t ew = wt == ARENA_BF16 ? 2 : 4, wbytes = (size_t)d * d * ew;
      d_wk_all.reserve(pf_n_full * wbytes, stream); d_wv_all.reserve(pf_n_full * wbytes, stream);
      d_bk_all.reserve((size_t)pf_n_full * d * 4, stream); d_bv_all.reserve((size_t)pf_n_full * d * 4, stream);
      int li = 0;
      for (const PfDecLayer& L : pdec) {
        if (!L.full) continue;
        HIP_CHECK(hipMemcpyAsync((unsigned char*)d_wk_all.ptr + li * wbytes, L.wkv, wbytes, hipMemcpyDeviceToDevice, stream));
        HIP_CHECK(hipMemcpyAsync((unsigned char*)d_wv_all.ptr + li * wbytes, (const unsigned char*)L.wkv + wbytes, wbytes, hipMemcpyDeviceToDevice, stream));
        HIP_CHECK(hipMemcpyAsync(d_bk_all.as<float>() + (size_t)li * d, L.bkv, (size_t)d * 4, hipMemcpyDeviceToDevice, stream));
        HIP_CHECK(hipMemcpyAsync(d_bv_all.as<float>() + (size_t)li * d, L.bkv + d, (size_t)d * 4, hipMemcpyDeviceToDevice, stream));
        ++li;
      }
    }
  }
  blocks.resize(c.n_blocks);
  for (int i = 0; i < c.n_blocks; ++i) {
    SvBlock& b = blocks[i];
    const std::string p = "blk" + std::to_string(i) + ".";
    b.kpad = (int)arena.get(p + "wqkv").shape[1];
    b.in_size = b.kpad == d ? d : feat;
    ASR_REQUIRE(b.kpad == round_up(b.in_size, 64), "sensevoice: block %d has K = %d", i, b.kpad);
    b.ln1_g = opt(p + "ln1_g", {b.in_size});
    b.ln1_b = opt(p + "ln1_b", {b.in_size});
    b.wqkv = arena.get(p + "wqkv", wt, {3 * d, b.kpad}).ptr;
    b.bqkv = (const float*)arena.get(p + "bqkv", ARENA_F32, {3 * d}).ptr;
    b.wfsmn = (const float*)arena.get(p + "wfsmn", ARENA_F32, {d, c.fsmn_kernel}).ptr;
    b.bfsmn = (const float*)arena.get(p + "bfsmn", ARENA_F32, {d}).ptr;
    b.wout = arena.get(p + "wout", wt, {d, d}).ptr;
    b.cqkv = opt(p + "cqkv", {3 * d});
    b.c1 = opt(p + "c1", {dff});
    b.ln2_g = opt(p + "ln2_g", {d});
    b.ln2_b = opt(p + "ln2_b", {d});
    b.w1 = arena.get(p + "w1", wt, {dff, d}).ptr;
    b.b1 = (const float*)arena.get(p + "b1", ARENA_F32, {dff}).ptr;
    b.w2 = arena.get(p + "w2", wt, {d, dff}).ptr;
    b.b2 = (const float*)arena.get(p + "b2", ARENA_F32, {d}).ptr;
  }
// ... 987 lines not shown
```

automatic-speech-recognition-asr-onnx_amd/csrc/whisper.hip:

```cpp
#include <cstdlib>
#include <cstring>

#include "../../include/asr_mi355x.h"
#include "decode_head.h"
#include "engine.h"
#include "gemm.h"
#include "kernels.h"

namespace {

inline int round_up(int v, int m) { return (v + m - 1) / m * m; }

template <typename T>
__global__ __launch_bounds__(256) void wh_beam_prompt_kernel(const T* __restrict__ pool, const int32_t* __restrict__ ptable, int pages_per_seq,
                                                             const T* __restrict__ kc, const T* __restrict__ vc, int max_pos, int B, int H, int p0, int beam,
                                                             int S, T* __restrict__ ext) {
  const int row = blockIdx.x, N = gridDim.x, lkh = blockIdx.y;
  const int h = lkh % H, kv = (lkh / H) & 1, l = lkh / (2 * H), b = row / beam;
  T* dst = ext + ((size_t)l * N + row) * 2 * H * S * 64 + ((size_t)kv * H + h) * S * 64;
  for (int i = threadIdx.x; i < p0 * 64; i += blockDim.x) {
    const int s = i >> 6, e = i & 63;
    const T* src = pool ? pool + (size_t)ptable[(size_t)b * pages_per_seq + (s >> 4)] * gridDim.y * 1024 + (size_t)lkh * 1024 + (size_t)(s & 15) * 64
                        : (kv ? vc : kc) + (((size_t)l * B + b) * H + h) * max_pos * 64 + (size_t)s * 64;
    dst[(size_t)s * 64 + e] = src[e];
// ... 17 lines not shown
  FrontEnd fe;
  std::vector<EncLayer> enc;
  std::vector<DecLayer> dec;
  const float *conv1_b = nullptr, *conv2_b = nullptr, *enc_pos = nullptr, *enc_ln_g = nullptr,
              *enc_ln_b = nullptr, *ckv_b = nullptr, *dec_pos = nullptr, *suppress = nullptr, *begin = nullptr, *dec_ln_g = nullptr,
              *dec_ln_b = nullptr;
  const void *conv1_w = nullptr, *conv2_w = nullptr, *ckv_w = nullptr, *embed = nullptr;
  int k_conv1 = 0;

  int batch = 0, rows = 0, Mpad = 0, hist = 0, max_T_enc = 0;
  std::vector<UttPlan> plan;
  DeviceBuffer d_plan, d_audio, d_mel, d_blkmax, d_x0, d_h1, d_xa, d_xb, d_xc, d_h, d_qk, d_vt, d_ctx, d_ffn, d_cross;
  DeviceBuffer d_kc, d_vc, d_ids, d_next, d_logits, d_dx, d_dqkv, d_dtok, d_hist;
  DeviceBuffer d_kstart;
  bool kstart_on = false;
  const int32_t* kstart() const { return kstart_on ? d_kstart.as<int32_t>() : nullptr; }
  static constexpr int KV_PAGE = 16;
  DeviceBuffer d_kvpool, d_ptable;
  bool kv_paged = true;
  int kv_gens = 0, kv_batch = 0, kv_shuffle = 0;
  void ensure_kv_pages(int B, int positions, size_t elem_bytes);
  TokenHead head;
  DeviceBuffer d_nsp;
  bool use_graph = true;
  bool use_decode_gemm = true;
  DeviceBuffer d_colsum, d_dlo;
  bool fp8_mm = false;
  int fp8_act_shift = 0;
  std::vector<Enc8Layer> enc8;
  DeviceBuffer d_ew8, d_ewscale, d_h8, d_ffn8, d_sat;
  bool fp4 = false;
  bool fp8 = false, fp8_fake = false, fp8_weights = true, fp8_kv = true;
  LowBitWeights dec8;
  DeviceBuffer d_cross8, d_cscale;
  StepGraph dec_graph;
  StepGraph beam_graph[2];
  DeviceBuffer d_bext, d_bhist, d_blogits;
  BeamRanker ranker;
  bool after_prefill = false;
  bool wts_on = false, wts_consumed = false;
  int wts_max_rows = 0, wts_p0 = -1, wts_ld = 0, wts_rows = 0;
  uint64_t wts_epoch = 0;
  std::vector<int32_t> wts_pairs;
  std::vector<int> wts_first, wts_count;
  std::vector<int32_t> wts_n_rows, wts_n_frames;
  DeviceBuffer d_wsel, d_wscores, d_wstats, d_wcost, d_wtrace, d_wn, d_wframes;
  PinnedBuffer h_walign;
  int n_pairs() const { return (int)wts_pairs.size() / 2; }
  void set_word_timestamps(int enable, const int32_t* pairs, int n, int max_rows);
  void align(const int32_t* n_rows, const int32_t* n_frames, int width, int32_t* frames_out, int out_stride);
  void align_read(int what, int b, void* host_out, size_t bytes, int32_t* shape_out);
  uint64_t ws_epoch = 1;
  PinnedBuffer h_plan, h_io;

  void init();
  SplitKGemm sk;
  void gemm(const GemmArgs& g) { sk.run(g, precision, stream); }
  template <typename T> void encode(const void* audio, int audio_mem, const int64_t* offs, int B, int32_t* n_pos_out);
  template <typename T> void enqueue_step(const int32_t* ids_dev, int n, bool is_prefill, bool use_hist_dev, const BeamStep* bs = nullptr, bool prompt = false);
  template <typename T> void step(const int32_t* ids_host, int n, bool is_prefill, int32_t* next_out, float* logits_out, const int32_t* pad_host = nullptr);
  void prefill_prompts(const int32_t* ids, const int32_t* offsets, int32_t* next_out, float* logits_out);
  template <typename T> void beam_search(int beam, int max_new, int eos_id, int32_t* tokens_out, int32_t* n_out, float* scores_out);
};

void WhSession::init() {
  const auto& c = cfg;
  ASR_REQUIRE(c.d_model == c.n_heads * c.d_head && c.d_head == 64, "whisper: head_dim must be 64 and d_model = heads * 64");
  ASR_REQUIRE(c.d_model % 128 == 0 && c.d_ffn % 128 == 0, "whisper: d_model and d_ffn must be multiples of 128");
  ASR_REQUIRE(c.nfft == 400 && c.hop_length == 160, "whisper: front-end is built for n_fft 400 / hop 160");
  ASR_REQUIRE(c.n_mels % 16 == 0, "whisper: n_mels must be a multiple of 16");
  ASR_REQUIRE(c.max_target_positions <= 1536, "whisper: decoder context too long for the attention kernel");
  vpad = round_up(c.vocab, 128);
  head.init(c.max_target_positions, 0, 20, 512);
  head.prof = &prof; ranker.prof = &prof;
  fe.init(c.nfft, c.nfft, c.hop_length, c.n_mels, 1, 1e-10f);
  model_rate = c.sample_rate;
  act = c.gelu_tanh ? ACT_GELU_TANH : ACT_GELU_ERF;
  const int wt = precision == ASR_PRECISION_BF16 ? ARENA_BF16 : ARENA_F32;
  const int d = c.d_model, dff = c.d_ffn, Ld = c.n_dec_layers;
  auto F = [&](const std::string& n, std::initializer_list<int64_t> sh) { return (const float*)arena.get(n, ARENA_F32, sh).ptr; };
  auto W = [&](const std::string& n, std::initializer_list<int64_t> sh) { return arena.get(n, wt, sh).ptr; };
  fe.dft = F("fe.dft", {(int64_t)fe.n_bin_tiles * 2 * fe.n_kchunks * 64 * 4});
  fe.melp = F("fe.mel", {(int64_t)(c.n_mels / 16) * fe.n_bin_tiles * 64 * 4});
  k_conv1 = round_up(3 * c.n_mels, 64);
  conv1_w = W("enc.conv1_w", {d, k_conv1});
  conv1_b = F("enc.conv1_b", {d});
  conv2_w = W("enc.conv2_w", {d, 3 * d});
  conv2_b = F("enc.conv2_b", {d});
  enc_pos = F("enc.pos", {c.max_source_positions, d});
  enc_ln_g = F("enc.ln_g", {d});
  enc_ln_b = F("enc.ln_b", {d});
  ckv_w = W("ckv.w", {2 * Ld * d, d});
  ckv_b = F("ckv.b", {2 * Ld * d});
  embed = W("dec.embed", {vpad, d});
  dec_pos = F("dec.pos", {c.max_target_positions, d});
  suppress = F("dec.suppress", {vpad});
  begin = F("dec.begin", {vpad});
  dec_ln_g = F("dec.ln_g", {d});
  dec_ln_b = F("dec.ln_b", {d});
  enc.resize(c.n_enc_layers);
  for (int i = 0; i < c.n_enc_layers; ++i) {
    const std::string p = "enc" + std::to_string(i) + ".";
    enc[i] = EncLayer{W(p + "wqkv", {3 * d, d}), W(p + "wo", {d, d}), W(p + "w1", {dff, d}), W(p + "w2", {d, dff}),
                      F(p + "bqkv", {3 * d}), F(p + "bo", {d}), F(p + "b1", {dff}), F(p + "b2", {d})};
  }
  dec.resize(Ld);
  for (int i = 0; i < Ld; ++i) {
    const std::string p = "dec" + std::to_string(i) + ".";
    dec[i] = DecLayer{W(p + "wqkv", {3 * d, d}), W(p + "wo", {d, d}), W(p + "wcq", {d, d}), W(p + "wco", {d, d}),
                      W(p + "w1", {dff, d}), W(p + "w2", {d, dff}),
                      F(p + "bqkv", {3 * d}), F(p + "bo", {d}), F(p + "bcq", {d}), F(p + "bco", {d}), F(p + "b1", {dff}), F(p + "b2", {d})};
  }
  if (fp8_mm) {
    ASR_REQUIRE(d % 256 == 0 && dff % 256 == 0, "whisper: FP8MM mode needs d_model and d_ffn to be multiples of 256");
    const size_t per = (size_t)2 * d * dff;
    d_ew8.reserve((size_t)c.n_enc_layers * per, stream); d_ewscale.reserve((size_t)c.n_enc_layers * (d + dff) * 4, stream);
    d_sat.reserve(8, stream); HIP_CHECK(hipMemsetAsync(d_sat.ptr, 0, 8, stream));
    enc8.resize(c.n_enc_layers);
    for (int i = 0; i < c.n_enc_layers; ++i) {
      unsigned char* w8 = d_ew8.as<unsigned char>() + i * per;
      float* sc = d_ewscale.as<float>() + (size_t)i * (d + dff);
      launch_quantize_rows_fp8((const bf16_t*)enc[i].w1, d, dff, d, w8, sc, nullptr, stream);
      launch_quantize_rows_fp8((const bf16_t*)enc[i].w2, dff, d, dff, w8 + (size_t)dff * d, sc + dff, nullptr, stream);
      enc8[i] = Enc8Layer{w8, w8 + (size_t)dff * d, sc, sc + dff};
    }
  }
  if (fp8 && fp8_weights) {
    ASR_REQUIRE(d % 256 == 0 && dff % 256 == 0, "whisper: FP8 / MXFP4 mode needs d_model and d_ffn to be multiples of 256");
    dec8.build(Ld, fp4, [&](int i) {
      DecLayer& L = dec[i];
      return std::vector<LowBitWeights::Slot>{{&L.wqkv, 3 * d, d}, {&L.wo, d, d}, {&L.wcq, d, d}, {&L.wco, d, d}, {&L.w1, dff, d}, {&L.w2, d, dff}};
    }, stream);
  }
  if (precision == ASR_PRECISION_BF16 && use_decode_gemm) {
    const size_t per = (size_t)3 * d + d + dff;
    d_colsum.reserve((size_t)Ld * per * 4, stream);
    for (int i = 0; i < Ld; ++i) {
      float* c0 = d_colsum.as<float>() + i * per;
      launch_colsum_bf16((const bf16_t*)dec[i].wqkv, d, 3 * d, d, c0, stream);
      launch_colsum_bf16((const bf16_t*)dec[i].wcq, d, d, d, c0 + 3 * d, stream);
      launch_colsum_bf16((const bf16_t*)dec[i].w1, d, dff, d, c0 + 4 * d, stream);
    }
    HIP_CHECK(hipStreamSynchronize(stream));
  }
}

template <typename T>
void WhSession::encode(const void* audio, int audio_mem, const int64_t* audio_offs, int B, int32_t* n_pos_out) {
  const auto& c = cfg;
  ASR_REQUIRE(B > 0 && audio && audio_offs, "whisper_encode: bad argument");
  HIP_CHECK(hipSetDevice(device));
  const AudioIn in = stage_input(*this, true, audio, audio_mem, audio_offs, B);
  const int64_t* const offs = in.offs;
  const int d = c.d_model, dff = c.d_ffn, Ld = c.n_dec_layers, H = c.n_heads;
  plan.assign(B, UttPlan{});
  std::vector<UttPlan> splan(B);
  int r = 0, rg = 0, frames = 0, n_fb = 0, n_qb = 0, max_T = 0;
  const int64_t base0 = offs[0];
  for (int b = 0; b < B; ++b) {
    UttPlan& p = plan[b];
    fe.plan_utt("whisper", b, offs, c.max_audio_len, p, frames, n_fb);
    p.T = (p.n_frames + 1) / 2;
    p.n_lfr = p.T;
    ASR_REQUIRE(p.T <= c.max_source_positions, "whisper: %d encoder positions exceed max_source_positions", p.T);
    p.row_off = r;
    splan[b] = p;
// ... 901 lines not shown
```

automatic-speech-recognition-asr-onnx_amd/engine.py:

```python
from __future__ import annotations

import ctypes as C
import warnings
from typing import Sequence

import numpy as np

from . import _lib
from .arena import PRECISION_BF16, PRECISION_F32, PRECISION_FP8MM, PRECISION_FP8W, PRECISION_MXFP4W, build_sensevoice_arena
from .config import SenseVoiceConfig

MEM_HOST, MEM_DEVICE = 0, 1
AUDIO_F32, AUDIO_I16, AUDIO_F16 = 0, 1, 2
AUDIO_DTYPE_NAMES = {"F32": np.dtype(np.float32), "INT16": np.dtype(np.int16), "F16": np.dtype(np.float16)}
_AUDIO_CODES = {np.dtype(np.float32): AUDIO_F32, np.dtype(np.int16): AUDIO_I16, np.dtype(np.float16): AUDIO_F16}


def audio_np_dtype(audio_dtype) -> np.dtype:
    if isinstance(audio_dtype, str):
        if audio_dtype not in AUDIO_DTYPE_NAMES:
            raise ValueError(f"input audio dtype {audio_dtype!r}: expected one of {sorted(AUDIO_DTYPE_NAMES)}")
        return AUDIO_DTYPE_NAMES[audio_dtype]
    dt = np.dtype(audio_dtype)
    if dt not in _AUDIO_CODES:
# ... 42 lines not shown
        return self._audio_np

    @audio_dtype.setter
    def audio_dtype(self, audio_dtype):
        dt = audio_np_dtype(audio_dtype)
        _lib.check(_lib.load().asr_session_set_audio_dtype(self._h, _AUDIO_CODES[dt]))
        self._audio_np = dt

    def _audio(self, a) -> np.ndarray:
        if self._audio_np == np.float32:
            return _f32(a)
        got = a.dtype if isinstance(a, np.ndarray) else np.asarray(a).dtype
        if got != self._audio_np:
            raise TypeError(f"{type(self).__name__}: the session's audio_dtype is {self._audio_np.name}, the audio given is {got.name} "
                            f"(convert it explicitly, or set audio_dtype)")
        return np.ascontiguousarray(a)

    @property
    def input_format(self) -> tuple[int, int]:
        rate, ch = C.c_int(0), C.c_int(0)
        _lib.check(_lib.load().asr_session_input_format(self._h, C.byref(rate), C.byref(ch)))
        return rate.value, ch.value

    def set_input_format(self, sample_rate: int, channels: int = 1):
        _lib.check(_lib.load().asr_session_set_input_format(self._h, int(sample_rate), int(channels)))
        self._format = self.input_format

    def model_lengths(self, frames) -> np.ndarray:
        n = np.asarray(frames, dtype=np.int64)
        rate, _ = self._format or (0, 1)
        model = int(self.cfg.sample_rate)
        if not rate or rate == model:
            return n
        g = int(np.gcd(rate, model))
        return -((-n * (model // g)) // (rate // g))

    def _pack(self, audios):
        ch = (self._format or (0, 1))[1]
        flat = [self._audio(a).reshape(-1) for a in audios]
        if any(a.size % ch for a in flat):
            raise ValueError(f"{type(self).__name__}: a clip's sample count is not a multiple of the {ch} interleaved channels of the input format")
        offs = np.zeros(len(flat) + 1, dtype=np.int64)
        offs[1:] = np.cumsum([a.size // ch for a in flat])
        return flat, np.concatenate(flat), offs

    def close(self):
        if self._h:
            _lib.check(_lib.load().asr_session_destroy(self._h))
            self._h = C.c_void_p(None)
        self._keep = None

    def __del__(self):
        try:
            self.close()
        except Exception:
            pass

    def set_stream(self, hip_stream: int):
        _lib.check(_lib.load().asr_session_set_stream(self._h, C.c_void_p(hip_stream)))

    def profile(self, enable: bool):
        _lib.check(_lib.load().asr_session_profile_enable(self._h, int(enable)))

    def profile_reset(self):
        _lib.check(_lib.load().asr_session_profile_reset(self._h))

    def profile_read(self) -> dict:
        cap = 64
        names = C.create_string_buffer(32 * cap)
        ms = (C.c_double * cap)()
        cnt = (C.c_int64 * cap)()
        n = C.c_int(0)
        _lib.check(_lib.load().asr_session_profile_read(self._h, cap, names, ms, cnt, C.byref(n)))
        out = {}
        for i in range(n.value):
            nm = names.raw[i * 32:(i + 1) * 32].split(b"\0", 1)[0].decode()
            out[nm] = {"total_ms": ms[i], "launches": int(cnt[i])}
        return out

    def sanm_stats(self) -> dict:
        out = np.zeros(8, dtype=np.int32)
        _lib.check(_lib.load().asr_sanm_stats(self._h, _ip(out)))
        return {"giveups": int(out[0]), "cooldown": int(out[1]), "foreign_diverted": int(out[2]), "block_kernel": bool(out[3])}

    def taps(self, enable: bool):
        _lib.check(_lib.load().asr_session_taps_enable(self._h, int(enable)))

    def tap(self, name: str, dtype=np.float32) -> np.ndarray:
        rows, cols = C.c_int64(0), C.c_int64(0)
        _lib.check(_lib.load().asr_session_tap_shape(self._h, name.encode(), C.byref(rows), C.byref(cols)))
        out = np.empty((rows.value, cols.value), dtype=dtype)
        _lib.check(_lib.load().asr_session_tap_read(self._h, name.encode(), out.ctypes.data_as(C.c_void_p), out.nbytes))
        return out


class SenseVoiceSession(_Session):

    def __init__(self, cfg: SenseVoiceConfig, arena, precision: int = PRECISION_BF16, device_id: int = 0,
                 arena_device_ptr: int | None = None, arena_bytes: int | None = None, audio_dtype=np.float32):
        super().__init__()
        self.cfg, self.precision, self.device_id = cfg, precision, device_id
        self._cfg_c = sensevoice_config_c(cfg)
        lib = _lib.load()
        if arena_device_ptr is not None:
            self._keep = arena
            _lib.check(lib.asr_sensevoice_create(C.byref(self._cfg_c), C.c_void_p(arena_device_ptr), arena_bytes, MEM_DEVICE,
                                                 device_id, precision, C.byref(self._h)))
        else:
            blob = np.ascontiguousarray(arena, dtype=np.uint8)
            _lib.check(lib.asr_sensevoice_create(C.byref(self._cfg_c), blob.ctypes.data_as(C.c_void_p), blob.nbytes, MEM_HOST,
                                                 device_id, precision, C.byref(self._h)))
        self.audio_dtype = audio_dtype

    @classmethod
    def from_checkpoint(cls, cfg, ck, precision=PRECISION_BF16, device_id=0, audio_dtype=np.float32):
        return cls(cfg, build_sensevoice_arena(cfg, ck, precision), precision, device_id, audio_dtype=audio_dtype)

    def seq_len(self, n_samples: int) -> int:
        return self.cfg.seq_len(n_samples)

    def run_packed(self, audio, offsets: np.ndarray, language_idx: np.ndarray, audio_device_ptr: int | None = None):
        offsets = np.ascontiguousarray(offsets, dtype=np.int64)
        lang = np.ascontiguousarray(language_idx, dtype=np.int32)
        B = lang.shape[0]
        assert offsets.shape[0] == B + 1
        max_t = max(self.cfg.seq_len(int(n)) for n in self.model_lengths(np.diff(offsets))) if B else 1
        tok = np.zeros((B, max_t), dtype=np.int32)
        num = np.zeros((B,), dtype=np.int32)
        lib = _lib.load()
        if audio_device_ptr is not None:
            ap, mem = C.c_void_p(audio_device_ptr), MEM_DEVICE
        else:
            audio = self._audio(audio).reshape(-1)
            ap, mem = audio.ctypes.data_as(C.c_void_p), MEM_HOST
        _lib.check(lib.asr_sensevoice_run(self._h, ap, mem, offsets.ctypes.data_as(C.POINTER(C.c_int64)), B, _ip(lang),
                                          _ip(tok), max_t, _ip(num)))
        return tok, num

    def run(self, audios: Sequence[np.ndarray], language_idx: Sequence[int]):
        flat, packed, offs = self._pack(audios)
        tok, num = self.run_packed(packed, offs, np.asarray(language_idx, dtype=np.int32))
        return [tok[b, :num[b]].copy() for b in range(len(flat))]

    def run_packed_timed(self, audio, offsets: np.ndarray, language_idx: np.ndarray, audio_device_ptr: int | None = None):
        offsets = np.ascontiguousarray(offsets, dtype=np.int64)
        lang = np.ascontiguousarray(language_idx, dtype=np.int32)
        B = lang.shape[0]
        assert offsets.shape[0] == B + 1
        max_t = max(self.cfg.seq_len(int(n)) for n in self.model_lengths(np.diff(offsets))) if B else 1
        tok = np.zeros((B, max_t), dtype=np.int32)
        first, last = np.zeros((B, max_t), dtype=np.int32), np.zeros((B, max_t), dtype=np.int32)
        logprob = np.zeros((B, max_t), dtype=np.float32)
        num = np.zeros((B,), dtype=np.int32)
        lib = _lib.load()
        if audio_device_ptr is not None:
            ap, mem = C.c_void_p(audio_device_ptr), MEM_DEVICE
        else:
            audio = self._audio(audio).reshape(-1)
            ap, mem = audio.ctypes.data_as(C.c_void_p), MEM_HOST
        _lib.check(lib.asr_sensevoice_run_timed(self._h, ap, mem, offsets.ctypes.data_as(C.POINTER(C.c_int64)), B, _ip(lang),
                                                _ip(tok), max_t, _ip(num), _ip(first), _ip(last), _fp(logprob)))
        return tok, num, first, last, logprob

    def run_timed(self, audios: Sequence[np.ndarray], language_idx: Sequence[int]):
        flat, packed, offs = self._pack(audios)
        tok, num, first, last, logprob = self.run_packed_timed(packed, offs, np.asarray(language_idx, dtype=np.int32))
# ... 53 lines not shown
        fi, ff = (0, 0.0) if fill is None else fill
        tids_c = tids if tids.size else np.zeros(1, np.int32)
        first, last = np.full(n, fi, dtype=np.int32), np.full(n, fi, dtype=np.int32)
        logprob = np.full(n, ff, dtype=np.float32)
        path, lik = np.zeros(B, dtype=np.float32), np.zeros(B, dtype=np.float32)
        status = np.zeros(B, dtype=np.int32)
        if audio_device_ptr is not None:
            ap, mem = C.c_void_p(audio_device_ptr), MEM_DEVICE
        else:
            audio = self._audio(audio).reshape(-1)
            ap, mem = audio.ctypes.data_as(C.c_void_p), MEM_HOST
        _lib.check(_lib.load().asr_sensevoice_align(self._h, ap, mem, offsets.ctypes.data_as(C.POINTER(C.c_int64)), B, _ip(lang), _ip(tids_c), _ip(toff),
                                                    _ip(first), _ip(last), _fp(logprob), _fp(path), _fp(lik), _ip(status)))
        return first[:tids.size], last[:tids.size], logprob[:tids.size], path, lik, status

    def align(self, audios: Sequence[np.ndarray], language_idx: Sequence[int], targets: Sequence[Sequence[int]]):
        flat, packed, offs = self._pack(audios)
        targets = [np.asarray(t, dtype=np.int32).reshape(-1) for t in targets]
        if len(targets) != len(flat):
            raise ValueError(f"align: {len(flat)} utterances, {len(targets)} transcripts")
        toff = np.zeros(len(targets) + 1, dtype=np.int32)
        toff[1:] = np.cumsum([t.size for t in targets])
        tids = np.concatenate(targets) if targets else np.zeros(0, np.int32)
        first, last, logprob, path, lik, status = self.align_packed(packed, offs, np.asarray(language_idx, dtype=np.int32), tids, toff)
        out = []
        for b in range(len(flat)):
            ok = status[b] == 0
            sl = slice(int(toff[b]), int(toff[b + 1]) if ok else int(toff[b]))
            out.append({"first_frame": first[sl].copy(), "last_frame": last[sl].copy(), "logprob": logprob[sl].copy(), "path_score": float(path[b]),
                        "loglik": float(lik[b]), "aligned": bool(ok)})
        return out

    def utterance_rows(self, lengths: Sequence[int]):
        out, r = [], 0
        for n in lengths:
            t = self.cfg.seq_len(int(n))
            out.append((r, t))
            r += (t + 15) // 16 * 16
        return out


def op_gemm(a, w, bias=None, act=0, precision=PRECISION_BF16):
    a, w = _f32(a), _f32(w)
    M, K = a.shape
    N = w.shape[0]
    out = np.empty((M, N), dtype=np.float32)
    b = _f32(bias) if bias is not None else None
    _lib.check(_lib.load().asr_op_gemm(precision, _fp(a), _fp(w), _fp(b), M, N, K, act, _fp(out)))
    return out


def op_gemm_ln(x, w, bias=None, gamma=None, beta=None):
    x, w = _f32(x), _f32(w)
    out = np.empty((x.shape[0], w.shape[0]), dtype=np.float32)
    b, g, be = (_f32(a) if a is not None else None for a in (bias, gamma, beta))
    _lib.check(_lib.load().asr_op_gemm_ln(_fp(x), _fp(w), _fp(b), _fp(g), _fp(be), x.shape[0], w.shape[0], x.shape[1], _fp(out)))
    return out


def op_layernorm(x, gamma=None, beta=None, eps=1e-5, precision=PRECISION_F32):
    x = _f32(x)
    rows, D = x.shape
    out = np.empty_like(x)
    g = _f32(gamma) if gamma is not None else None
    b = _f32(beta) if beta is not None else None
    _lib.check(_lib.load().asr_op_layernorm(precision, _fp(x), rows, D, _fp(g), _fp(b), eps, _fp(out)))
    return out


def op_attention(q, k, v, seq_lens, n_heads, d_head, precision=PRECISION_BF16):
    q, k, v = _f32(q), _f32(k), _f32(v)
    sl = np.ascontiguousarray(seq_lens, dtype=np.int32)
    out = np.empty_like(q)
    _lib.check(_lib.load().asr_op_attention(precision, _fp(q), _fp(k), _fp(v), _ip(sl), sl.size, n_heads, d_head, _fp(out)))
    return out


def op_fsmn(v, w, b, seq_lens, precision=PRECISION_F32):
    v, w, b = _f32(v), _f32(w), _f32(b)
    sl = np.ascontiguousarray(seq_lens, dtype=np.int32)
    out = np.empty_like(v)
    _lib.check(_lib.load().asr_op_fsmn(precision, _fp(v), _fp(w), _fp(b), _ip(sl), sl.size, v.shape[1], w.shape[1], _fp(out)))
    return out


def resample_table(sample_rate: int, model_rate: int = 16000):
    L, M, W = C.c_int(0), C.c_int(0), C.c_int(0)
    lib = _lib.load()
    _lib.check(lib.asr_resample_table(int(sample_rate), int(model_rate), C.byref(L), C.byref(M), C.byref(W), None))
    coeffs = np.empty((L.value, 2 * W.value + 1), dtype=np.float32)
    _lib.check(lib.asr_resample_table(int(sample_rate), int(model_rate), C.byref(L), C.byref(M), C.byref(W), _fp(coeffs)))
    return L.value, M.value, W.value, coeffs


def op_resample(audio, offsets, sample_rate: int, model_rate: int = 16000, channels: int = 1, int16_scale: bool = False):
    audio = np.ascontiguousarray(audio).reshape(-1)
    code = _AUDIO_CODES[audio_np_dtype(audio.dtype)]
    offs = np.ascontiguousarray(offsets, dtype=np.int64)
    if offs.size < 2 or np.any(np.diff(offs) < 0) or offs[0] < 0 or int(offs[-1]) * int(channels) > audio.size:
        raise ValueError("op_resample: offsets must be non-decreasing frame offsets inside the audio given")
    L, M, W = C.c_int(0), C.c_int(0), C.c_int(0)
    _lib.check(_lib.load().asr_resample_table(int(sample_rate), int(model_rate), C.byref(L), C.byref(M), C.byref(W), None))
    n_out = -((-np.diff(offs) * L.value) // M.value)
    out = np.empty(max(int(n_out.sum()), 1), dtype=np.float32)
    offs_out = np.zeros(offs.size, dtype=np.int64)
    lp = C.POINTER(C.c_int64)
    _lib.check(_lib.load().asr_op_resample(audio.ctypes.data_as(C.c_void_p), offs.ctypes.data_as(lp), offs.size - 1, code, int(sample_rate), int(model_rate),
                                           int(channels), int(bool(int16_scale)), _fp(out), out.size, offs_out.ctypes.data_as(lp)))
    return out[:int(offs_out[-1])], offs_out


def op_ctc_collapse(frame_ids, seq_lens, blank_id=0):
    ids = np.ascontiguousarray(frame_ids, dtype=np.int32)
    sl = np.ascontiguousarray(seq_lens, dtype=np.int32)
    max_t = int(sl.max())
    tok = np.zeros((sl.size, max_t), dtype=np.int32)
    num = np.zeros((sl.size,), dtype=np.int32)
    _lib.check(_lib.load().asr_op_ctc_collapse(_ip(ids), _ip(sl), sl.size, blank_id, _ip(tok), max_t, _ip(num)))
    return [tok[b, :num[b]].copy() for b in range(sl.size)]


def op_ctc_collapse_timed(frame_ids, frame_logprob, seq_lens, blank_id=0, max_tokens=None, fill=None):
    ids = np.ascontiguousarray(frame_ids, dtype=np.int32)
    lp = _f32(frame_logprob)
    sl = np.ascontiguousarray(seq_lens, dtype=np.int32)
    assert ids.size == lp.size == int(sl.sum())
    max_t = int(sl.max()) if max_tokens is None else int(max_tokens)
    fi, ff = (0, 0.0) if fill is None else fill
    tok, first, last = (np.full((sl.size, max_t), fi, dtype=np.int32) for _ in range(3))
    tlp = np.full((sl.size, max_t), ff, dtype=np.float32)
    num = np.zeros((sl.size,), dtype=np.int32)
    _lib.check(_lib.load().asr_op_ctc_collapse_timed(_ip(ids), _fp(lp), _ip(sl), sl.size, blank_id, _ip(tok), _ip(first), _ip(last), _fp(tlp), max_t,
                                                     _ip(num)))
    return tok, first, last, tlp, num


def hotword_trie(phrases):
    kids, depth, is_end = [{}], [0], [0]
    for ph in phrases:
        ph = [int(t) for t in ph]
        if not ph:
            raise ValueError("empty hotword phrase")
        n = 0
        for t in ph:
            if t not in kids[n]:
                kids[n][t] = len(kids)
                kids.append({})
                depth.append(depth[n] + 1)
                is_end.append(0)
            n = kids[n][t]
        is_end[n] = 1
    order, remap = [0], {0: 0}
    for n in order:
        for t in sorted(kids[n]):
            remap[kids[n][t]] = len(order)
            order.append(kids[n][t])
    off, tok, node = [0], [], []
    for n in order:
        for t in sorted(kids[n]):
            tok.append(t)
            node.append(remap[kids[n][t]])
        off.append(len(tok))
    i32 = lambda a: np.asarray(a, dtype=np.int32)
    return {"depth": i32([depth[n] for n in order]), "is_end": i32([is_end[n] for n in order]), "child_off": i32(off), "child_tok": i32(tok),
            "child_node": i32(node)}

# ... 872 lines not shown
```

include/asr_mi355x.h:

```cpp
#ifndef ASR_MI355X_H
#define ASR_MI355X_H

#include <stddef.h>
#include <stdint.h>

#ifdef __cplusplus
extern "C" {
#endif

#define ASR_ABI_VERSION 1

enum asr_status {
  ASR_STATUS_OK = 0,
  ASR_STATUS_INVALID = 1,
  ASR_STATUS_HIP = 2,
  ASR_STATUS_NOT_FOUND = 3,
  ASR_STATUS_UNSUPPORTED = 4,
  ASR_STATUS_NO_DEVICE = 5
};

enum asr_precision { ASR_PRECISION_BF16 = 0, ASR_PRECISION_F32 = 1, ASR_PRECISION_FP8W = 2, ASR_PRECISION_FP8MM = 3, ASR_PRECISION_MXFP4W = 4 };

enum asr_mem { ASR_MEM_HOST = 0, ASR_MEM_DEVICE = 1 };

// ... 85 lines not shown
                                      float* pend_am_out, int32_t* total_out);
int asr_paraformer_stream_stats(asr_session* s, int32_t* out8);

typedef struct asr_whisper_config {
  int32_t sample_rate, n_mels, nfft, hop_length;
  int32_t d_model, n_heads, d_head, d_ffn, n_enc_layers, n_dec_layers;
  int32_t vocab, max_source_positions, max_target_positions, max_audio_len;
  int32_t gelu_tanh;
  int32_t reserved[9];
} asr_whisper_config;

int asr_whisper_create(const asr_whisper_config* cfg, const void* arena, size_t arena_bytes, int arena_mem, int device_id,
                       int precision, asr_session** out);
int asr_whisper_encode(asr_session* s, const void* audio, int audio_mem, const int64_t* audio_offsets, int batch,
                       int32_t* n_positions_out);
int asr_whisper_prefill(asr_session* s, const int32_t* ids, int n, int32_t* next_ids_out, float* logits_out);
int asr_whisper_prefill_prompts(asr_session* s, const int32_t* ids, const int32_t* offsets, int32_t* next_ids_out, float* logits_out);
int asr_whisper_decode(asr_session* s, const int32_t* ids, int32_t* next_ids_out, float* logits_out);
int asr_whisper_generate(asr_session* s, int max_new, int eos_id, int32_t* tokens_out, int32_t* n_out);
int asr_whisper_beam_search(asr_session* s, int beam, int max_new, int eos_id, int32_t* tokens_out, int32_t* n_out, float* scores_out);
int asr_whisper_set_penalty(asr_session* s, float repeat_penalty, int penalty_range);
int asr_whisper_set_fp8_act_shift(asr_session* s, int shift);
int asr_whisper_fp8_stats(asr_session* s, uint64_t stats[2]);

int asr_whisper_track_history(asr_session* s, int enable);
int asr_whisper_no_speech_prob(asr_session* s, int no_speech_id, float* prob_out);
int asr_whisper_set_sampling(asr_session* s, int enable, float temperature, int top_k, float top_p, float repetition_penalty,
                             uint64_t seed);
int asr_whisper_set_sampling_noise(asr_session* s, const float* uniforms, int count);
int asr_whisper_set_token_scores(asr_session* s, int enable);
int asr_whisper_set_hotwords(asr_session* s, const int32_t* ids, const int32_t* offsets, int n_phrases, float boost);
int asr_whisper_set_lm(asr_session* s, const int32_t* image_words, int64_t n_words, float alpha, float beta, float oov_logprob, int topk,
                       const int32_t* end_ids, int n_end_ids);
int asr_whisper_token_scores(asr_session* s, float* logprob_out, int out_stride, int32_t* n_out);
int asr_whisper_set_timestamps(asr_session* s, int enable, int timestamp_begin_id, int no_timestamps_id, int eot_id, int max_initial_index);
int asr_whisper_set_word_timestamps(asr_session* s, int enable, const int32_t* layer_head_pairs, int n_pairs, int max_rows);
int asr_whisper_align(asr_session* s, const int32_t* n_rows, const int32_t* n_frames, int medfilt_width, int32_t* token_frames_out, int out_stride);
int asr_whisper_align_read(asr_session* s, int what, int b, void* host_out, size_t bytes, int32_t* shape_out);

typedef struct asr_qwen_config {
  int32_t sample_rate, n_mels, nfft, hop_length;
  int32_t enc_d, enc_heads, enc_ffn, n_enc_layers, conv_channels, n_window, n_window_infer, max_source_positions;
  int32_t d_model, n_heads, n_kv_heads, d_head, d_ffn, n_layers, vocab, max_seq_len, max_audio_len;
  float rms_eps, rope_theta;
  int32_t classify_num;
  int32_t reserved[8];
} asr_qwen_config;

int asr_qwen_create(const asr_qwen_config* cfg, const void* arena, size_t arena_bytes, int arena_mem, int device_id, int precision,
                    asr_session** out);
int asr_qwen_prefill(asr_session* s, const void* audio, int audio_mem, const int64_t* audio_offsets, int batch, const int32_t* pre_ids,
                     const int32_t* pre_offsets, const int32_t* post_ids, const int32_t* post_offsets, int32_t* next_ids_out, float* logits_out,
                     int32_t* ids_len_out);
int asr_qwen_decode(asr_session* s, const int32_t* ids, int32_t* next_ids_out, float* logits_out);
int asr_qwen_set_penalty(asr_session* s, float repeat_penalty, int penalty_range);
int asr_qwen_track_history(asr_session* s, int enable);
int asr_qwen_set_sampling(asr_session* s, int enable, float temperature, int top_k, float top_p, float repetition_penalty, uint64_t seed);
int asr_qwen_set_sampling_noise(asr_session* s, const float* uniforms, int count);
int asr_qwen_set_token_scores(asr_session* s, int enable);
int asr_qwen_set_hotwords(asr_session* s, const int32_t* ids, const int32_t* offsets, int n_phrases, float boost);
int asr_qwen_set_lm(asr_session* s, const int32_t* image_words, int64_t n_words, float alpha, float beta, float oov_logprob, int topk, const int32_t* end_ids,
                    int n_end_ids);
int asr_qwen_token_scores(asr_session* s, float* logprob_out, int out_stride, int32_t* n_out);
int asr_qwen_generate(asr_session* s, int max_new, const int32_t* stop_ids, int n_stop, int32_t* tokens_out, int32_t* n_out);
int asr_qwen_kv_stats(asr_session* s, int32_t* out4);
int asr_qwen_beam_search(asr_session* s, int beam, int max_new, const int32_t* stop_ids, int n_stop, int32_t* tokens_out, int32_t* n_out,
                         float* scores_out);

int asr_qwen_align(asr_session* s, const void* audio, int audio_mem, const int64_t* audio_offsets, int batch, const int32_t* pre_ids,
                   const int32_t* pre_offsets, const int32_t* post_ids, const int32_t* post_offsets, int32_t timestamp_id, int32_t* slot_offsets_out,
                   int32_t* buckets_out, int64_t buckets_cap, float* logits_out, int32_t* ids_len_out);

int asr_mem_alloc(int device_id, size_t bytes, void** out);
int asr_mem_free(int device_id, void* ptr);
int asr_mem_copy(int device_id, void* dst, const void* src, size_t bytes, int kind);

int asr_session_destroy(asr_session* s);
int asr_session_set_stream(asr_session* s, void* hip_stream);
int asr_session_device(asr_session* s, int* device_id);
int asr_session_set_audio_dtype(asr_session* s, int audio_dtype);
int asr_session_audio_dtype(asr_session* s, int* audio_dtype_out);
int asr_session_set_input_format(asr_session* s, int sample_rate, int channels);
int asr_session_input_format(asr_session* s, int* sample_rate_out, int* channels_out);

int asr_session_profile_enable(asr_session* s, int enable);
int asr_session_profile_reset(asr_session* s);
int asr_session_profile_read(asr_session* s, int cap, char* names, double* total_ms, int64_t* launches, int* n_out);

int asr_session_taps_enable(asr_session* s, int enable);
int asr_session_tap_shape(asr_session* s, const char* name, int64_t* rows, int64_t* cols);
int asr_session_tap_read(asr_session* s, const char* name, void* host_out, size_t bytes);

int asr_op_gemm(int precision, const float* a, const float* w, const float* bias, int M, int N, int K, int act,
                float* out);
int asr_op_layernorm(int precision, const float* x, int rows, int D, const float* gamma, const float* beta, float eps,
                     float* out);
int asr_op_attention(int precision, const float* q, const float* k, const float* v, const int32_t* seq_lens, int batch,
                     int n_heads, int d_head, float* ctx);
int asr_op_fsmn(int precision, const float* v, const float* w, const float* b, const int32_t* seq_lens, int batch,
                int channels, int ktaps, float* out);
int asr_op_gemm_ln(const float* x, const float* w, const float* bias, const float* gamma, const float* beta, int M, int N, int K,
                   float* out);
int asr_op_ctc_collapse(const int32_t* frame_ids, const int32_t* seq_lens, int batch, int blank_id, int32_t* token_ids,
                        int max_tokens, int32_t* num_id);
int asr_op_ctc_collapse_timed(const int32_t* frame_ids, const float* frame_logprob, const int32_t* seq_lens, int batch, int blank_id,
                              int32_t* token_ids, int32_t* first_frame, int32_t* last_frame, float* token_logprob, int max_tokens, int32_t* num_id);
int asr_op_ctc_prefix_beam(const int32_t* cand_id, const float* cand_logprob, int topk, const int32_t* seq_lens, int batch, int blank_id,
                           const int32_t* trie_depth, const int32_t* trie_is_end, const int32_t* trie_child_off, const int32_t* trie_child_tok,
                           const int32_t* trie_child_node, int n_nodes, float boost, int beam, int nbest, int32_t* token_ids, int max_tokens,
                           int32_t* num_id, float* score, float* ctc_score);
int asr_op_ctc_prefix_beam_lm(const int32_t* cand_id, const float* cand_logprob, int topk, const int32_t* seq_lens, int batch, int blank_id,
                              const int32_t* trie_depth, const int32_t* trie_is_end, const int32_t* trie_child_off, const int32_t* trie_child_tok,
                              const int32_t* trie_child_node, int n_nodes, float boost, int beam, int nbest, int32_t* token_ids, int max_tokens,
                              int32_t* num_id, float* score, float* ctc_score, const int32_t* lm_image, int64_t lm_words, float alpha, float beta,
                              float oov_logprob);
int asr_op_nar_beam(const int32_t* cand_id, const float* cand_logprob, int topk, const int32_t* seq_lens, int batch, const int32_t* trie_depth,
                    const int32_t* trie_is_end, const int32_t* trie_child_off, const int32_t* trie_child_tok, const int32_t* trie_child_node, int n_nodes,
                    float boost, const int32_t* lm_image, int64_t lm_words, float alpha, float beta, float oov_logprob, int beam, int nbest,
                    int32_t* token_ids, int max_tokens, int32_t* num_id, float* score, float* am_score, float* token_logprob);
int asr_nar_stream_beam_state_words(int beam, int pend_cap);
int asr_op_nar_stream_beam(const int32_t* cand_id, const float* cand_logprob, int topk, int n_streams, int n_steps, const int32_t* step_off,
                           const int32_t* slot_stream, const int32_t* slot_rows, const int32_t* slot_final, const int32_t* trie_depth,
                           const int32_t* trie_is_end, const int32_t* trie_child_off, const int32_t* trie_child_tok, const int32_t* trie_child_node,
                           int n_nodes, float boost, const int32_t* lm_image, int64_t lm_words, float alpha, float beta, float oov_logprob, int beam,
                           int nbest, int pend_cap, int32_t* state_io, int state_words, int32_t* commit_ids, float* commit_logprob, int commit_cap,
                           int32_t* commit_num, int32_t* pend_ids, float* pend_logprob, int32_t* pend_num, float* pend_score, float* pend_am,
                           int32_t* total);
int asr_op_ctc_align(const float* em, int ld_em, const int32_t* seq_lens, int batch, int row0, const int32_t* target_ids, const int32_t* target_offsets,
                     int32_t* first_frame, int32_t* last_frame, float* token_logprob, int max_tokens, float* path_score, float* loglik, int32_t* status);
int asr_op_cif_scan_timed(const float* alpha, const float* enc, int d, const int32_t* seq_lens, int batch, float tail_threshold, float* acoustic_out,
                          int32_t* fire_frame_out, int max_tokens, int32_t* num_id_out);
int asr_op_resample(const void* audio, const int64_t* offsets, int batch, int audio_dtype, int rate_in, int rate_model, int channels, int int16_scale,
                    float* out, int64_t out_cap, int64_t* offsets_out);
int asr_resample_table(int rate_in, int rate_model, int* L, int* M, int* W, float* coeffs);

#ifdef __cplusplus
}
#endif
#endif
```

Before: 77210 audio-s/s.

## Skip zero mel-filterbank tiles and dead DFT bin tiles in the fbank kernel

At session load the mel filter matrix is scanned once on the host to build liveness tables: which DFT bin tiles feed any mel bin, and which (mel tile, bin tile) pairs are nonzero. Mel tiles are split between two wave groups with a balanced assignment. The split fbank kernel then computes DFT only for live bin tiles, runs the mel projection only over nonzero pairs, and templates on the number of valid 16-frame tiles so tail blocks issue fewer MFMAs. Tail blocks are also moved to the end of the block list. This removes redundant MFMA work in the front end, at the cost of more complex per-wave indexing and code specialisation. The front end is only a small part of a 70-block encoder, so end-to-end impact is bounded.

```diff
diff --git a/automatic-speech-recognition-asr-onnx_amd/_lib.py b/automatic-speech-recognition-asr-onnx_amd/_lib.py
--- a/automatic-speech-recognition-asr-onnx_amd/_lib.py
+++ b/automatic-speech-recognition-asr-onnx_amd/_lib.py
@@ -126,6 +126,8 @@
     "asr_session_audio_dtype": (_i, [_vp, C.POINTER(C.c_int)]),
     "asr_session_set_input_format": (_i, [_vp, _i, _i]),
     "asr_session_input_format": (_i, [_vp, C.POINTER(C.c_int), C.POINTER(C.c_int)]),
+    "asr_session_fbank_live": (_i, [_vp, _ip]),
+    "asr_fbank_live_tables": (_i, [_fp, _i, _i, _i, _ip, _i]),
     "asr_session_profile_enable": (_i, [_vp, _i]),
     "asr_session_profile_reset": (_i, [_vp]),
     "asr_session_profile_read": (_i, [_vp, _i, C.c_char_p, _dp, _lp, C.POINTER(C.c_int)]),
diff --git a/automatic-speech-recognition-asr-onnx_amd/csrc/api.hip b/automatic-speech-recognition-asr-onnx_amd/csrc/api.hip
--- a/automatic-speech-recognition-asr-onnx_amd/csrc/api.hip
+++ b/automatic-speech-recognition-asr-onnx_amd/csrc/api.hip
@@ -85,6 +85,23 @@
   return asr_guard([&] {
     ASR_REQUIRE(s && audio_dtype_out, "audio_dtype: null argument");
     *audio_dtype_out = s->audio_dtype;
+  });
+}
+
+extern "C" int asr_session_fbank_live(asr_session* s, int32_t* out4) {
+  return asr_guard([&] {
+    ASR_REQUIRE(s && out4, "fbank_live: null argument");
+    for (int i = 0; i < 4; ++i) out4[i] = s->fbank_live[i];
+  });
+}
+
+extern "C" int asr_fbank_live_tables(const float* mel_packed, int n_mel_tiles, int n_bin_tiles, int all_live, int32_t* words_out, int words_cap) {
+  return asr_guard([&] {
+    ASR_REQUIRE(mel_packed && words_out, "fbank_live_tables: null argument");
+    ASR_REQUIRE(words_cap >= (int)(sizeof(FbankLive) / 4), "fbank_live_tables: words_out holds %d words, the tables have %d", words_cap, (int)(sizeof(FbankLive) / 4));
+    FbankLive L;
+    fbank_live_build(mel_packed, n_mel_tiles, n_bin_tiles, all_live != 0, &L);
+    memcpy(words_out, &L, sizeof(FbankLive));
   });
 }
 
diff --git a/automatic-speech-recognition-asr-onnx_amd/csrc/engine.h b/automatic-speech-recognition-asr-onnx_amd/csrc/engine.h
--- a/automatic-speech-recognition-asr-onnx_amd/csrc/engine.h
+++ b/automatic-speech-recognition-asr-onnx_amd/csrc/engine.h
@@ -192,6 +192,7 @@
   size_t audio_elt() const { return audio_dtype == 0 ? 4 : 2; }
   int model_rate = 16000;
   int in_rate = 0, in_channels = 1;
+  int32_t fbank_live[4] = {0, 0, 0, 0};
   Resampler resampler;
   hipStream_t stream = nullptr;
   bool own_stream = false;
@@ -209,6 +210,9 @@
   int n_bin_tiles = 0, n_kchunks = 0, n_mels = 0, win = 0, hop = 0, whisper = 0;
   float log_floor = 0.0f;
   void init(int nfft, int win_, int hop_, int n_mels_, int whisper_, float log_floor_);
+  FbankLive live = {};
+  DeviceBuffer d_live;
+  void build_live(asr_session& s);
   void plan_utt(const char* family, int b, const int64_t* offs, int max_audio_len, UttPlan& p, int& frames, int& n_fb) const;
   FbankArgs args(const void* audio, int audio_dtype, const UttPlan* plan, const int32_t* blk_utt, const int32_t* blk_f0, float* mel_out, float* blk_max) const;
 };
diff --git a/automatic-speech-recognition-asr-onnx_amd/csrc/engine.hip b/automatic-speech-recognition-asr-onnx_amd/csrc/engine.hip
--- a/automatic-speech-recognition-asr-onnx_amd/csrc/engine.hip
+++ b/automatic-speech-recognition-asr-onnx_amd/csrc/engine.hip
@@ -276,12 +276,29 @@
   fa.mel_out = mel_out; fa.n_bin_tiles = n_bin_tiles; fa.n_kchunks = n_kchunks; fa.n_mel_tiles = n_mels / 16; fa.n_mels = n_mels;
   fa.win = win; fa.hop = hop; fa.log_floor = log_floor; fa.whisper = whisper; fa.blk_max = blk_max; fa.dft_split = dft_split;
   fa.log_at_floor = (float)(whisper ? std::log10((double)log_floor) : std::log((double)log_floor));
+  fa.live = d_live.as<FbankLive>();
   return fa;
 }
 
+void FrontEnd::build_live(asr_session& s) {
+  ASR_REQUIRE(melp && n_bin_tiles > 0 && n_mels % 16 == 0, "front end: the liveness tables need the mel matrix");
+  const int n_mel_tiles = n_mels / 16;
+  std::vector<float> host((size_t)n_mel_tiles * n_bin_tiles * 256);
+  HIP_CHECK(hipMemcpyAsync(host.data(), melp, host.size() * 4, hipMemcpyDeviceToHost, s.stream));
+  HIP_CHECK(hipStreamSynchronize(s.stream));
+  fbank_live_build(host.data(), n_mel_tiles, n_bin_tiles, !env_flag("ASR_FBANK_LIVE", true), &live);
+  d_live.reserve(sizeof(FbankLive), s.stream);
+  HIP_CHECK(hipMemcpyAsync(d_live.ptr, &live, sizeof(FbankLive), hipMemcpyHostToDevice, s.stream));
+  HIP_CHECK(hipStreamSynchronize(s.stream));
+  s.fbank_live[0] = live.n_bt; s.fbank_live[1] = n_bin_tiles; s.fbank_live[2] = live.n_pairs; s.fbank_live[3] = n_mel_tiles * n_bin_tiles;
+}
+
 void fill_fbank_blocks(const UttPlan* plan, int B, int32_t* blk_utt, int32_t* blk_f0) {
-  for (int b = 0, i = 0; b < B; ++b)
-    for (int f0 = 0; f0 < plan[b].n_frames; f0 += 64) { blk_utt[i] = b; blk_f0[i++] = f0; }
+  int i = 0;
+  for (int b = 0; b < B; ++b)
+    for (int f0 = 0; f0 + 64 <= plan[b].n_frames; f0 += 64) { blk_utt[i] = b; blk_f0[i++] = f0; }
+  for (int b = 0; b < B; ++b)
+    if (plan[b].n_frames % 64) { blk_utt[i] = b; blk_f0[i++] = plan[b].n_frames / 64 * 64; }
 }
 void fill_query_blocks(const UttPlan* plan, int n, int q_rows, int32_t* qb_utt, int32_t* qb_q0) {
   for (int u = 0, i = 0; u < n; ++u)
diff --git a/automatic-speech-recognition-asr-onnx_amd/csrc/kernels.h b/automatic-speech-recognition-asr-onnx_amd/csrc/kernels.h
--- a/automatic-speech-recognition-asr-onnx_amd/csrc/kernels.h
+++ b/automatic-speech-recognition-asr-onnx_amd/csrc/kernels.h
@@ -18,6 +18,18 @@
 
 enum { AUDIO_F32 = 0, AUDIO_I16 = 1, AUDIO_F16 = 2 };
 inline size_t audio_elt_bytes(int audio_dtype) { return audio_dtype == AUDIO_F32 ? 4 : 2; }
+constexpr int FB_MAX_BIN_TILES = 17, FB_MAX_MEL_TILES = 16;
+struct FbankLive {
+  int32_t n_bin_tiles, n_mel_tiles;
+  int32_t n_bt;
+  int32_t n_pairs;
+  int32_t all_frames;
+  int32_t n_grp[2];
+  int32_t bt[FB_MAX_BIN_TILES];
+  int32_t grp[2][FB_MAX_MEL_TILES];
+  uint32_t mel_mask[FB_MAX_MEL_TILES];
+};
+void fbank_live_build(const float* mel_packed, int n_mel_tiles, int n_bin_tiles, bool all_live, FbankLive* out);
 struct FbankArgs {
   const void* audio;
   const UttPlan* plan;
@@ -37,6 +49,7 @@
   float* blk_max;
   const void* dft_split = nullptr;
   float log_at_floor = 0.0f;
+  const FbankLive* live = nullptr;
   int audio_dtype = AUDIO_F32;
 };
 void launch_fbank(const FbankArgs& a, int n_blocks, hipStream_t s);
diff --git a/automatic-speech-recognition-asr-onnx_amd/csrc/kernels.hip b/automatic-speech-recognition-asr-onnx_amd/csrc/kernels.hip
--- a/automatic-speech-recognition-asr-onnx_amd/csrc/kernels.hip
+++ b/automatic-speech-recognition-asr-onnx_amd/csrc/kernels.hip
@@ -117,7 +117,7 @@
     wmax = wave_max(wmax);
     if (lane == 0) red[wave] = wmax;
     __syncthreads();
-    if (tid == 0) a.blk_max[blockIdx.x] = fmaxf(fmaxf(red[0], red[1]), fmaxf(red[2], red[3]));
+    if (tid == 0) a.blk_max[up.blk0 + f0 / FB_FRAMES] = fmaxf(fmaxf(red[0], red[1]), fmaxf(red[2], red[3]));
   }
 }
 
@@ -174,107 +174,166 @@
   union BF { uint4 q; bf16x8_t v; };
   BF ring[FB_PF][6];
   const int wv = __builtin_amdgcn_readfirstlane(wave);
-  const int n_steps = (wv < a.n_bin_tiles && !(a.dbg & 1)) ? (a.n_bin_tiles - wv + FB_WAVES - 1) / FB_WAVES * FB_K32 : 0;
+  const FbankLive* __restrict__ lv = a.live;
+  auto tbl = [](const int32_t& x) { return __builtin_amdgcn_readfirstlane(x); };
+  const int n_bt = tbl(lv->n_bt);
+  const int n_mt = tbl(lv->all_frames) ? 4 : __builtin_amdgcn_readfirstlane(min(4, (up.n_frames - f0 + 15) >> 4));
+  static_assert(FB_MAX_BIN_TILES <= 3 * FB_WAVES, "a wave holds the ids of at most three bin tiles");
+  int my_t[3];
+#pragma unroll
+  for (int z = 0; z < 3; ++z) my_t[z] = tbl(lv->bt[max(min(wv + z * FB_WAVES, n_bt - 1), 0)]);
+  auto my_tile = [&](int i) { return i == 0 ? my_t[0] : i == 1 ? my_t[1] : my_t[2]; };
+  const int n_steps = (wv < n_bt && !(a.dbg & 1)) ? (n_bt - wv + FB_WAVES - 1) / FB_WAVES * FB_K32 : 0;
   constexpr size_t FB_IM = (size_t)FB_K32 * 3 * 64;
   auto frag_ptr = [&](int t, int kc) { return tab + (((size_t)(t * 2) * FB_K32 + kc) * 3) * 64 + lane; };
-  int pt = wv, pkc = 0, ps = 0;
+  int pti = 0, pkc = 0, ps = 0;
   auto refill = [&](BF (&slot)[6]) {
-    const uint4* src = frag_ptr(pt, pkc);
+    const uint4* src = frag_ptr(my_tile(pti), pkc);
 #pragma unroll
     for (int z = 0; z < 3; ++z) { slot[z].q = src[z * 64]; slot[3 + z].q = src[FB_IM + z * 64]; }
-    if (ps + 1 < n_steps) { ++ps; if (++pkc == FB_K32) { pkc = 0; pt += FB_WAVES; } }
+    if (ps + 1 < n_steps) { ++ps; if (++pkc == FB_K32) { pkc = 0; ++pti; } }
   };
-  f32x4_t re[4], im[4];
-#pragma unroll
-  for (int mt = 0; mt < 4; ++mt) { re[mt] = f32x4_t{0.f, 0.f, 0.f, 0.f}; im[mt] = f32x4_t{0.f, 0.f, 0.f, 0.f}; }
-  if (n_steps > 0) {
-#pragma unroll
-    for (int u = 0; u < FB_PF; ++u) refill(ring[u]);
-  }
-  int t = wv, kc = 0;
-  for (int s0 = 0; s0 < n_steps; s0 += FB_PF) {
-#pragma unroll
-    for (int u = 0; u < FB_PF; ++u) {
-      if (s0 + u < n_steps) {
-        const int k = kc * 32 + fgrp * 8;
-        const int koff = k + ((k >= HOP) + (k >= 2 * HOP)) * 8;
-        bf16x8_t ah[4], al[4];
-#pragma unroll
-        for (int mt = 0; mt < 4; ++mt) {
-          const int pos = (mt * 16 + frow) * FB_HP + koff;
-          ah[mt] = *reinterpret_cast<const bf16x8_t*>(audh + pos); al[mt] = *reinterpret_cast<const bf16x8_t*>(audl + pos);
+  auto dft_steps = [&](auto n_mt_c) {
+    constexpr int NMT = decltype(n_mt_c)::value;
+    if (n_steps > 0) {
+#pragma unroll
+      for (int u = 0; u < FB_PF; ++u) refill(ring[u]);
+    }
+    f32x4_t re[NMT], im[NMT];
+#pragma unroll
+    for (int mt = 0; mt < NMT; ++mt) { re[mt] = f32x4_t{0.f, 0.f, 0.f, 0.f}; im[mt] = f32x4_t{0.f, 0.f, 0.f, 0.f}; }
+    int ti = 0, kc = 0;
+    for (int s0 = 0; s0 < n_steps; s0 += FB_PF) {
+#pragma unroll
+      for (int u = 0; u < FB_PF; ++u) {
+        if (s0 + u < n_steps) {
+          const int k = kc * 32 + fgrp * 8;
+          const int koff = k + ((k >= HOP) + (k >= 2 * HOP)) * 8;
+          bf16x8_t ah[NMT], al[NMT];
+#pragma unroll
+          for (int mt = 0; mt < NMT; ++mt) {
+            const int pos = (mt * 16 + frow) * FB_HP + koff;
+            ah[mt] = *reinterpret_cast<const bf16x8_t*>(audh + pos); al[mt] = *reinterpret_cast<const bf16x8_t*>(audl + pos);
+          }
+#define ASR_FB_TERM(X, ZR, ZI)                                                                          \
+          _Pragma("unroll") for (int mt = 0; mt < NMT; ++mt) {                                             \
+            re[mt] = __builtin_amdgcn_mfma_f32_16x16x32_bf16(X[mt], ring[u][ZR].v, re[mt], 0, 0, 0);       \
+            im[mt] = __builtin_amdgcn_mfma_f32_16x16x32_bf16(X[mt], ring[u][ZI].v, im[mt], 0, 0, 0);       \
+          }
+          ASR_FB_TERM(al, 1, 4)
+          ASR_FB_TERM(ah, 2, 5)
+          ASR_FB_TERM(al, 0, 3)
+          ASR_FB_TERM(ah, 1, 4)
+          ASR_FB_TERM(ah, 0, 3)
+#undef ASR_FB_TERM
+          if (++kc == FB_K32) {
+            const int t = my_tile(ti);
+#pragma unroll
+            for (int mt = 0; mt < NMT; ++mt) {
+#pragma unroll
+              for (int r = 0; r < 4; ++r)
+                pw[(mt * 16 + fgrp * 4 + r) * FB_PLD + t * 16 + frow] = re[mt][r] * re[mt][r] + im[mt][r] * im[mt][r];
+              re[mt] = f32x4_t{0.f, 0.f, 0.f, 0.f}; im[mt] = f32x4_t{0.f, 0.f, 0.f, 0.f};
+            }
+            kc = 0; ++ti;
+          }
         }
-#define ASR_FB_TERM(X, ZR, ZI)                                                                          \
-        _Pragma("unroll") for (int mt = 0; mt < 4; ++mt) {                                               \
-          re[mt] = __builtin_amdgcn_mfma_f32_16x16x32_bf16(X[mt], ring[u][ZR].v, re[mt], 0, 0, 0);       \
-          im[mt] = __builtin_amdgcn_mfma_f32_16x16x32_bf16(X[mt], ring[u][ZI].v, im[mt], 0, 0, 0);       \
-        }
-        ASR_FB_TERM(al, 1, 4)
-        ASR_FB_TERM(ah, 2, 5)
-        ASR_FB_TERM(al, 0, 3)
-        ASR_FB_TERM(ah, 1, 4)
-        ASR_FB_TERM(ah, 0, 3)
-#undef ASR_FB_TERM
-        if (++kc == FB_K32) {
-#pragma unroll
-          for (int mt = 0; mt < 4; ++mt) {
-#pragma unroll
-            for (int r = 0; r < 4; ++r)
-              pw[(mt * 16 + fgrp * 4 + r) * FB_PLD + t * 16 + frow] = re[mt][r] * re[mt][r] + im[mt][r] * im[mt][r];
-            re[mt] = f32x4_t{0.f, 0.f, 0.f, 0.f}; im[mt] = f32x4_t{0.f, 0.f, 0.f, 0.f};
-          }
-          kc = 0; t += FB_WAVES;
-        }
-      }
-      __builtin_amdgcn_sched_barrier(0);
-      if (!(a.dbg & 8)) refill(ring[u]);
-      __builtin_amdgcn_sched_barrier(0);
-    }
-  }
-  __syncthreads();
+        __builtin_amdgcn_sched_barrier(0);
+        if (!(a.dbg & 8)) refill(ring[u]);
+        __builtin_amdgcn_sched_barrier(0);
+      }
+    }
+  };
+  if (n_mt == 4) dft_steps(std::integral_constant<int, 4>{});
+  else if (n_mt == 3) dft_steps(std::integral_constant<int, 3>{});
+  else if (n_mt == 2) dft_steps(std::integral_constant<int, 2>{});
+  else dft_steps(std::integral_constant<int, 1>{});
 
   float wmax = -INFINITY;
   const float4* melp = reinterpret_cast<const float4*>(a.mel_packed);
   constexpr int FB_MT = 4;
-  const int fw = wave & 3, mg = wave >> 2;
-  for (int nt0 = mg; nt0 < ((a.dbg & 2) ? 0 : a.n_mel_tiles); nt0 += 2 * FB_MT) {
-    f32x4_t acc[FB_MT];
-#pragma unroll
-    for (int q = 0; q < FB_MT; ++q) acc[q] = f32x4_t{0.f, 0.f, 0.f, 0.f};
-    auto mel_frags = [&](float4 (&b)[FB_MT], int kc) {
-#pragma unroll
-      for (int q = 0; q < FB_MT; ++q) b[q] = nt0 + 2 * q < a.n_mel_tiles ? melp[(size_t)((nt0 + 2 * q) * a.n_bin_tiles + kc) * 64 + lane] : make_float4(0.f, 0.f, 0.f, 0.f);
-    };
-    float4 b4[FB_MT], b4n[FB_MT];
-    mel_frags(b4, 0);
-    for (int kc = 0; kc < a.n_bin_tiles; ++kc) {
-      mel_frags(b4n, kc + 1 < a.n_bin_tiles ? kc + 1 : kc);
-#pragma unroll
-      for (int j = 0; j < 4; ++j) {
-        const float av = pw[(fw * 16 + frow) * FB_PLD + kc * 16 + j * 4 + fgrp];
-#pragma unroll
-        for (int q = 0; q < FB_MT; ++q) {
-          const float bv = j == 0 ? b4[q].x : j == 1 ? b4[q].y : j == 2 ? b4[q].z : b4[q].w;
-          if (nt0 + 2 * q < a.n_mel_tiles) acc[q] = __builtin_amdgcn_mfma_f32_16x16x4f32(av, bv, acc[q], 0, 0, 0);
+  const int fw = wv & 3, mg = wv >> 2;
+  const int n_my = (fw < n_mt && !(a.dbg & 2)) ? tbl(lv->n_grp[mg]) : 0;
+  const int bt0 = tbl(lv->bt[0]);
+  constexpr int FB_MR = 3;
+  int nt[FB_MT], len[FB_MT], kcur[FB_MT], kring[FB_MR][FB_MT];
+  uint32_t left[FB_MT];
+  float4 mring[FB_MR][FB_MT];
+  auto next_frag = [&](int q, float4& b, int& k) {
+    if (left[q]) { kcur[q] = __builtin_ctz(left[q]); left[q] &= left[q] - 1; }
+    k = kcur[q];
+    b = melp[(size_t)(nt[q] * a.n_bin_tiles + k) * 64 + lane];
+  };
+  auto open_pass = [&](int g0) {
+#pragma unroll
+    for (int q = 0; q < FB_MT; ++q) {
+      const bool has = g0 + q < n_my;
+      nt[q] = has ? tbl(lv->grp[mg][min(g0 + q, FB_MAX_MEL_TILES - 1)]) : 0;
+      left[q] = has ? (uint32_t)tbl((const int32_t&)lv->mel_mask[nt[q]]) : 0u;
+      len[q] = __builtin_popcount(left[q]);
+      kcur[q] = bt0;
+    }
+#pragma unroll
+    for (int u = 0; u < FB_MR; ++u)
+#pragma unroll
+      for (int q = 0; q < FB_MT; ++q) {
+        kring[u][q] = bt0;
+        if (g0 + q < n_my) next_frag(q, mring[u][q], kring[u][q]);
+      }
+  };
+  if (n_my > 0) open_pass(0);
+  __syncthreads();
+
+  auto mel_pass = [&](int g0, auto nq_c) {
+    constexpr int NQ = decltype(nq_c)::value;
+    f32x4_t acc[NQ];
+    int n_it = 0;
+#pragma unroll
+    for (int q = 0; q < NQ; ++q) { acc[q] = f32x4_t{0.f, 0.f, 0.f, 0.f}; n_it = max(n_it, len[q]); }
+    for (int i0 = 0; i0 < n_it; i0 += FB_MR) {
+#pragma unroll
+      for (int u = 0; u < FB_MR; ++u) {
+        const int i = i0 + u;
+        if (i < n_it) {
+#pragma unroll
+          for (int j = 0; j < 4; ++j) {
+#pragma unroll
+            for (int q = 0; q < NQ; ++q) {
+              const float4& b = mring[u][q];
+              const float bw = j == 0 ? b.x : j == 1 ? b.y : j == 2 ? b.z : b.w;
+              const float bv = i < len[q] ? bw : 0.0f;
+              const float av = pw[(fw * 16 + frow) * FB_PLD + kring[u][q] * 16 + j * 4 + fgrp];
+              acc[q] = __builtin_amdgcn_mfma_f32_16x16x4f32(av, bv, acc[q], 0, 0, 0);
+            }
+          }
         }
-      }
-#pragma unroll
-      for (int q = 0; q < FB_MT; ++q) b4[q] = b4n[q];
-    }
-#pragma unroll
-    for (int q = 0; q < FB_MT; ++q) {
-      if (nt0 + 2 * q >= a.n_mel_tiles) continue;
+        __builtin_amdgcn_sched_barrier(0);
+#pragma unroll
+        for (int q = 0; q < NQ; ++q) next_frag(q, mring[u][q], kring[u][q]);
+        __builtin_amdgcn_sched_barrier(0);
+      }
+    }
+#pragma unroll
+    for (int q = 0; q < NQ; ++q) {
 #pragma unroll
       for (int r = 0; r < 4; ++r) {
         const int f = f0 + fw * 16 + fgrp * 4 + r;
         if (f < up.n_frames) {
           const float c = fmaxf(acc[q][r], a.log_floor);
           const float v = c <= a.log_floor ? a.log_at_floor : a.whisper ? log10f(c) : logf(c);
-          a.mel_out[(size_t)(up.frame_off + f) * a.n_mels + (nt0 + 2 * q) * 16 + frow] = v;
+          a.mel_out[(size_t)(up.frame_off + f) * a.n_mels + nt[q] * 16 + frow] = v;
           wmax = fmaxf(wmax, v);
         }
       }
     }
+  };
+  for (int g0 = 0; g0 < n_my; g0 += FB_MT) {
+    if (g0 > 0) open_pass(g0);
+    const int nq = n_my - g0;
+    if (nq >= 4) mel_pass(g0, std::integral_constant<int, 4>{});
+    else if (nq == 3) mel_pass(g0, std::integral_constant<int, 3>{});
+    else if (nq == 2) mel_pass(g0, std::integral_constant<int, 2>{});
+    else mel_pass(g0, std::integral_constant<int, 1>{});
   }
   if (a.whisper) {
     __shared__ float red[FB_WAVES];
@@ -285,7 +344,7 @@
       float m = red[0];
 #pragma unroll
       for (int w = 1; w < FB_WAVES; ++w) m = fmaxf(m, red[w]);
-      a.blk_max[blockIdx.x] = m;
+      a.blk_max[up.blk0 + f0 / FB_FRAMES] = m;
     }
   }
 }
@@ -1614,6 +1673,8 @@
     HIP_CHECK(hipFuncSetAttribute(reinterpret_cast<const void*>(fbank_kernel<S>), hipFuncAttributeMaxDynamicSharedMemorySize, (int)lds));
   }
   if (a.dft_split) {
+    ASR_REQUIRE(a.live, "fbank: the split kernel needs the session's liveness tables");
+    ASR_REQUIRE(a.n_mel_tiles <= FB_MAX_MEL_TILES, "fbank: too many mel bins");
     FbankArgs b = a;
     b.dbg = env_int("ASR_FBANK_DBG", b.dbg);
     const size_t lds2 = (size_t)FB_A16 * 2 * 2 + (size_t)FB_FRAMES * FB_PLD * sizeof(float);
@@ -1635,6 +1696,52 @@
     case AUDIO_F16: return launch_fbank_typed<_Float16>(a, n_blocks, s);
     default: ASR_THROW(ASR_ERR_INVALID, "fbank: unknown audio sample type %d", a.audio_dtype);
   }
+}
+
+void fbank_live_build(const float* mel_packed, int n_mel_tiles, int n_bin_tiles, bool all_live, FbankLive* out) {
+  ASR_REQUIRE(mel_packed && out, "fbank liveness: null argument");
+  ASR_REQUIRE(n_bin_tiles >= 1 && n_bin_tiles <= FB_MAX_BIN_TILES && n_mel_tiles >= 1 && n_mel_tiles <= FB_MAX_MEL_TILES,
+              "fbank liveness: %d mel tiles x %d bin tiles (at most %d x %d)", n_mel_tiles, n_bin_tiles, FB_MAX_MEL_TILES, FB_MAX_BIN_TILES);
+  FbankLive L = {};
+  L.n_bin_tiles = n_bin_tiles; L.n_mel_tiles = n_mel_tiles; L.all_frames = all_live ? 1 : 0;
+  uint32_t any = 0;
+  int pairs[FB_MAX_MEL_TILES] = {};
+  for (int nt = 0; nt < n_mel_tiles; ++nt) {
+    for (int kc = 0; kc < n_bin_tiles; ++kc) {
+      bool live = all_live;
+      const float* w = mel_packed + (size_t)(nt * n_bin_tiles + kc) * 256;
+      for (int i = 0; i < 256 && !live; ++i) live = w[i] != 0.0f;
+      if (live) { L.mel_mask[nt] |= 1u << kc; ++pairs[nt]; ++L.n_pairs; }
+    }
+    any |= L.mel_mask[nt];
+  }
+  for (int kc = 0; kc < n_bin_tiles; ++kc)
+    if ((any >> kc) & 1) L.bt[L.n_bt++] = kc;
+  uint32_t to1 = 0;
+  if (all_live) {
+    for (int nt = 0; nt < n_mel_tiles; ++nt) to1 |= (uint32_t)(nt & 1) << nt;
+  } else {
+    auto cost = [&](uint32_t set) {
+      int c = 0, in_pass = 0, longest = 0;
+      for (int nt = 0; nt < n_mel_tiles; ++nt) {
+        if (!((set >> nt) & 1)) continue;
+        longest = std::max(longest, pairs[nt]);
+        if (++in_pass == 4) { c += 4 * longest; in_pass = 0; longest = 0; }
+      }
+      return c + in_pass * longest;
+    };
+    const uint32_t all = (1u << n_mel_tiles) - 1;
+    const int cap = (n_mel_tiles + 1) / 2;
+    int best_max = INT32_MAX, best_sum = INT32_MAX;
+    for (uint32_t set = 0; set <= all; ++set) {
+      const int n1 = __builtin_popcount(set);
+      if (n1 > cap || n_mel_tiles - n1 > cap) continue;
+      const int c0 = cost(all & ~set), c1 = cost(set), mx = std::max(c0, c1);
+      if (mx < best_max || (mx == best_max && c0 + c1 < best_sum)) { best_max = mx; best_sum = c0 + c1; to1 = set; }
+    }
+  }
+  for (int nt = 0; nt < n_mel_tiles; ++nt) { const int g = (to1 >> nt) & 1; L.grp[g][L.n_grp[g]++] = nt; }
+  *out = L;
 }
 
 size_t fbank_split_table_bytes(int n_bin_tiles, int win) {
diff --git a/automatic-speech-recognition-asr-onnx_amd/csrc/qwen.hip b/automatic-speech-recognition-asr-onnx_amd/csrc/qwen.hip
--- a/automatic-speech-recognition-asr-onnx_amd/csrc/qwen.hip
+++ b/automatic-speech-recognition-asr-onnx_amd/csrc/qwen.hip
@@ -662,6 +662,7 @@
   auto W = [&](const std::string& n, std::initializer_list<int64_t> sh) { return arena.get(n, wt, sh).ptr; };
   fe.dft = F("fe.dft", {(int64_t)fe.n_bin_tiles * 2 * fe.n_kchunks * 64 * 4});
   fe.melp = F("fe.mel", {(int64_t)(c.n_mels / 16) * fe.n_bin_tiles * 64 * 4});
+  fe.build_live(*this);
   conv1_w = W("enc.conv1_w", {cpad, 64});          conv1_b = F("enc.conv1_b", {cpad});
   conv2_w = W("enc.conv2_w", {cpad, 9 * cpad});    conv2_b = F("enc.conv2_b", {cpad});
   conv3_w = W("enc.conv3_w", {cpad, 9 * cpad});    conv3_b = F("enc.conv3_b", {cpad});
diff --git a/automatic-speech-recognition-asr-onnx_amd/csrc/sensevoice.hip b/automatic-speech-recognition-asr-onnx_amd/csrc/sensevoice.hip
--- a/automatic-speech-recognition-asr-onnx_amd/csrc/sensevoice.hip
+++ b/automatic-speech-recognition-asr-onnx_amd/csrc/sensevoice.hip
@@ -33,6 +33,7 @@
     fe.dft_split = d_dft_split.ptr;
   }
   fe.melp = (const float*)arena.get("fe.mel", ARENA_F32, {(int64_t)(c.n_mels / 16) * fe.n_bin_tiles * 64 * 4}).ptr;
+  fe.build_live(*this);
   cmvn_means = opt("fe.cmvn_means", {feat});
   cmvn_vars = (const float*)arena.get("fe.cmvn_vars", ARENA_F32, {feat}).ptr;
   speech_pos = (const float*)arena.get("fe.speech_pos", ARENA_F32, {max_lfr, feat}).ptr;
diff --git a/automatic-speech-recognition-asr-onnx_amd/csrc/whisper.hip b/automatic-speech-recognition-asr-onnx_amd/csrc/whisper.hip
--- a/automatic-speech-recognition-asr-onnx_amd/csrc/whisper.hip
+++ b/automatic-speech-recognition-asr-onnx_amd/csrc/whisper.hip
@@ -123,6 +123,7 @@
   auto W = [&](const std::string& n, std::initializer_list<int64_t> sh) { return arena.get(n, wt, sh).ptr; };
   fe.dft = F("fe.dft", {(int64_t)fe.n_bin_tiles * 2 * fe.n_kchunks * 64 * 4});
   fe.melp = F("fe.mel", {(int64_t)(c.n_mels / 16) * fe.n_bin_tiles * 64 * 4});
+  fe.build_live(*this);
   k_conv1 = round_up(3 * c.n_mels, 64);
   conv1_w = W("enc.conv1_w", {d, k_conv1});
   conv1_b = F("enc.conv1_b", {d});
diff --git a/automatic-speech-recognition-asr-onnx_amd/engine.py b/automatic-speech-recognition-asr-onnx_amd/engine.py
--- a/automatic-speech-recognition-asr-onnx_amd/engine.py
+++ b/automatic-speech-recognition-asr-onnx_amd/engine.py
@@ -148,6 +148,11 @@
         out = np.zeros(8, dtype=np.int32)
         _lib.check(_lib.load().asr_sanm_stats(self._h, _ip(out)))
         return {"giveups": int(out[0]), "cooldown": int(out[1]), "foreign_diverted": int(out[2]), "block_kernel": bool(out[3])}
+
+    def fbank_live(self) -> dict:
+        out = np.zeros(4, dtype=np.int32)
+        _lib.check(_lib.load().asr_session_fbank_live(self._h, _ip(out)))
+        return {"live_bin_tiles": int(out[0]), "bin_tiles": int(out[1]), "live_pairs": int(out[2]), "pairs": int(out[3])}
 
     def taps(self, enable: bool):
         _lib.check(_lib.load().asr_session_taps_enable(self._h, int(enable)))
@@ -367,6 +372,19 @@
     out = np.empty_like(v)
     _lib.check(_lib.load().asr_op_fsmn(precision, _fp(v), _fp(w), _fp(b), _ip(sl), sl.size, v.shape[1], w.shape[1], _fp(out)))
     return out
+
+
+def fbank_live_tables(mel_packed, n_mel_tiles: int, n_bin_tiles: int, all_live: bool = False) -> dict:
+    m = _f32(mel_packed).reshape(-1)
+    if m.size != n_mel_tiles * n_bin_tiles * 256:
+        raise ValueError("fbank_live_tables: mel_packed must hold n_mel_tiles * n_bin_tiles fragments of 64 x 4 weights")
+    w = np.zeros(72, dtype=np.int32)
+    _lib.check(_lib.load().asr_fbank_live_tables(_fp(m), int(n_mel_tiles), int(n_bin_tiles), int(bool(all_live)), _ip(w), w.size))
+    n_bt, n_grp = int(w[2]), (int(w[5]), int(w[6]))
+    grp = w[24:56].reshape(2, 16)
+    return {"n_bin_tiles": int(w[0]), "n_mel_tiles": int(w[1]), "live_pairs": int(w[3]), "all_frames": bool(w[4]),
+            "bin_tiles": w[7:7 + n_bt].tolist(), "wave_mel_tiles": [grp[g, :n_grp[g]].tolist() for g in range(2)],
+            "mel_masks": w[56:56 + int(w[1])].view(np.uint32).tolist()}
 
 
 def resample_table(sample_rate: int, model_rate: int = 16000):
diff --git a/include/asr_mi355x.h b/include/asr_mi355x.h
--- a/include/asr_mi355x.h
+++ b/include/asr_mi355x.h
@@ -191,6 +191,9 @@
 int asr_session_audio_dtype(asr_session* s, int* audio_dtype_out);
 int asr_session_set_input_format(asr_session* s, int sample_rate, int channels);
 int asr_session_input_format(asr_session* s, int* sample_rate_out, int* channels_out);
+
+int asr_session_fbank_live(asr_session* s, int32_t* out4);
+int asr_fbank_live_tables(const float* mel_packed, int n_mel_tiles, int n_bin_tiles, int all_live, int32_t* words_out, int words_cap);
 
 int asr_session_profile_enable(asr_session* s, int enable);
 int asr_session_profile_reset(asr_session* s);
```

Result: no change. 77550 audio-s/s, median of 6 (+0.4%).
